# endernewton/tf-faster-rcnn

Hardware: AMD Instinct MI355X
Metric: images/sec (600×1000) ResNet-101 Faster R-CNN at 1/2/4/8 MI355X (higher is better)
Workload: dtype f32 (operands, accumulators, results; GEMMs with Cin, Cout % 128 == 0 form each f32 product from two-piece fp16 operands with an exact power-of-two scale per 128-k block on the fp16 matrix pipe -- 3 MFMAs / product, dropped terms <= 3 * 2^-22, measured error vs float64 below the f32-MFMA kernel's; o

## Files before the change

### include/frcnn_hip.h

```cpp
#ifndef FRCNN_HIP_H_
#define FRCNN_HIP_H_
#include <stddef.h>
#include <stdint.h>

#ifdef __cplusplus
extern "C" {
#endif

#define FRCNN_OK 0
#define FRCNN_E_ARG (-1)
#define FRCNN_E_WS (-2)
#define FRCNN_E_UNSUPPORTED (-3)
#define FRCNN_E_HIP(e) (-(1000 + (int)(e)))

#define FRCNN_NMS_RULE_CPU 0
#define FRCNN_NMS_RULE_GPU 1

#define FRCNN_ACT_NONE 0
#define FRCNN_ACT_RELU 1
#define FRCNN_ACT_RELU6 2

#define FRCNN_ABI_VERSION 6
int frcnn_abi_version(void);
const char* frcnn_build_info(void);
// ... 115 lines not shown
int frcnn_proposal_recall_host(const float* boxes, int box_stride, long long n_rows, const long long* start, const int* count,
                               const float* scale, int n_images, long long max_boxes, int limit, const double* gt,
                               const long long* gt_off, long long n_gt_total, double* gt_iou, int* ran_out, void* ws, size_t ws_bytes);

int frcnn_conv2d_nhwc(const float* x_d, int N, int H, int W, int Cin, const float* w_d, const float* bias_d,
                      const float* residual_d, int RH, int RW, int res_stride, float* y_d, int OH, int OW,
                      int Cout, int KH, int KW, int stride, int pad_top, int pad_left, int act, int fold_w,
                      void* stream);
size_t frcnn_conv2d_workspace_bytes(int N, int OH, int OW, int Cout, int KH, int KW, int Cin, int fold_w);
int frcnn_conv2d_nhwc_ws(const float* x_d, int N, int H, int W, int Cin, const float* w_d, const float* bias_d,
                         const float* residual_d, int RH, int RW, int res_stride, float* y_d, int OH, int OW, int Cout, int KH,
                         int KW, int stride, int pad_top, int pad_left, int act, int fold_w, void* ws, size_t ws_bytes,
                         void* stream);

int frcnn_set_tuning(int key, int value);
unsigned int frcnn_crc32c(const void* data, size_t n, unsigned int crc);

long long frcnn_snappy_uncompress(const unsigned char* src, size_t n, unsigned char* dst, size_t cap);

int frcnn_prep_image_shape(int h, int w, int target_size, int max_size, double* im_scale, int* out_h, int* out_w);
int frcnn_prep_image(const void* src_d, int src_is_float, int h, int w, const double* pixel_means, double im_scale, float* out_d,
                     int OH, int OW, int out_c, void* stream);
int frcnn_prep_image_batched(const void* src_d, int src_is_float, int B, int h, int w, const double* pixel_means, double im_scale,
                             float* out_d, int OH, int OW, int out_c, void* stream);
int frcnn_prep_train_image(const void* src_d, int src_is_float, int h, int w, int flipped, const double* pixel_means, double im_scale,
                           float* out_d, int OH, int OW, int out_c, const unsigned short* boxes_d, const int* classes_d, int G,
                           float* gt_d, void* stream);

int frcnn_jpeg_info(const unsigned char* data, size_t n, int* out8);
size_t frcnn_jpeg_coef_bytes(int width, int height, int ncomp, int hs, int vs);
int frcnn_jpeg_entropy_decode(const unsigned char* data, size_t n, void* coef_h, size_t coef_bytes);
int frcnn_jpeg_pixels_host(const void* coef_h, int width, int height, int ncomp, int hs, int vs, unsigned char* bgr_h);
size_t frcnn_jpeg_workspace_bytes(int width, int height, int ncomp, int hs, int vs);
int frcnn_jpeg_pixels(const void* coef_d, int width, int height, int ncomp, int hs, int vs, unsigned char* bgr_d, void* ws,
                      size_t ws_bytes, void* stream);

int frcnn_jpeg_quant_tables(int quality, unsigned short* out128);
int frcnn_jpeg_coefs(const unsigned char* bgr_d, int width, int height, int hs, int vs, int quality, void* coef_d, void* ws,
                     size_t ws_bytes, void* stream);
int frcnn_jpeg_coefs_host(const unsigned char* bgr_h, int width, int height, int hs, int vs, int quality, void* coef_h);
size_t frcnn_jpeg_stream_bound(int width, int height, int hs, int vs);
long long frcnn_jpeg_entropy_encode(const void* coef_h, int width, int height, int hs, int vs, unsigned char* out, size_t cap);

int frcnn_draw_detections(unsigned char* bgr_d, int h, int w, const float* dets_d, const int* cnt_d, int max_dets, float conf,
                          int thickness, int scale, const unsigned char* colours_d, int num_colours, const unsigned char* labels_d,
                          int num_classes, int label_stride, const unsigned char* glyphs_d, void* stream);
int frcnn_draw_detections_host(unsigned char* bgr_h, int h, int w, const float* dets_h, int count, int max_dets, float conf,
                               int thickness, int scale, const unsigned char* colours_h, int num_colours, const unsigned char* labels_h,
                               int num_classes, int label_stride, const unsigned char* glyphs_h);

int frcnn_gemm_batched_nt(const float* x_d, const float* w_d, float* y_d, int G, int M, int N, int K, void* stream);
size_t frcnn_gemm_x3_pack_bytes(int G, int N, int K);
int frcnn_gemm_x3_pack(const float* w_d, int G, int N, int K, void* planes_d, void* stream);
int frcnn_gemm_x3(const float* x_d, const void* planes_d, const float* bias_d, const float* res_d, float* y_d, int G, int M, int N,
                  int K, int act, int cfg, int terms, void* stream);
size_t frcnn_h2_planes_bytes(long long rows, int K);
int frcnn_h2_pack_w(const float* w_d, int G, int N, int K, void* planes_d, float* w_inv_d, void* stream);
int frcnn_h2_split(const float* x_d, long long M, int K, void* planes_d, float* inv_d, void* stream);
int frcnn_gemm_h2(const void* x_planes_d, const float* x_inv_d, const void* w_planes_d, const float* w_inv_d, const float* bias_d,
                  const float* res_d, const void* res_planes_d, const float* res_inv_d, float* y_d, void* y_planes_d, float* y_inv_d,
                  int G, int M, int N, int K, int act, int cfg, void* stream);
size_t frcnn_gemm_h2_mean_workspace_bytes(int G, int M, int N);
int frcnn_gemm_h2_mean(const void* x_planes_d, const float* x_inv_d, const void* w_planes_d, const float* w_inv_d, const float* bias_d,
                       const float* res_d, const void* res_planes_d, const float* res_inv_d, int G, int M, int N, int K, int act, int rows,
                       float* mean_out_d, void* ws, size_t ws_bytes, int cfg, void* stream);
int frcnn_winograd_filter_transform(const float* w_hwio, int Cin, int Cout, const float* scale, int m, float* u_out);
int frcnn_winograd_filter_transform_device(const float* w_packed_d, int Cout, int Cin, int m, int transpose_flip, float* u_d,
                                           void* stream);
int frcnn_winograd_input_transform(const float* x_d, int N, int H, int W, int C, int m, float* v_d, void* stream);
int frcnn_winograd_output_transform(const float* m_d, int N, int H, int W, int C, int m, const float* bias_d, int act, float* y_d,
                                    void* stream);
int frcnn_winograd2_conv_x3(const float* x_d, int N, int H, int W, const void* u_planes_d, const float* bias_d, int act, float* y_d,
                            void* stream);
int frcnn_winograd7_filter_transform(const float* w_hwio, int Cin, int Cout, const float* scale, float* u_out);
int frcnn_winograd7_filter_transform_device(const float* w_packed_d, int Cout, int Cin, int transpose_flip, float* u_d, void* stream);
int frcnn_winograd7_input_transform(const float* x_d, int R, int C, float* v_d, void* stream);
int frcnn_winograd7_output_transform(const float* m_d, int R, int C, const float* bias_d, int act, float* y_d, void* stream);
int frcnn_winograd_input_transform_h2(const float* x_d, int N, int H, int W, int C, int m, void* v_planes_d, float* v_inv_d, void* stream);
int frcnn_winograd_output_transform_h2(const float* m_d, int N, int H, int W, int C, int m, const float* bias_d, int act, float* y_d,
                                       void* y_planes_d, float* y_inv_d, void* stream);
int frcnn_winograd7_input_transform_h2(const float* x_d, int R, int C, void* v_planes_d, float* v_inv_d, void* stream);
int frcnn_winograd7_output_transform_h2(const float* m_d, int R, int C, const float* bias_d, int act, float* y_d, void* y_planes_d,
                                        float* y_inv_d, void* stream);
int frcnn_pack_filter_hwio(const float* w_hwio, int KH, int KW, int Cin, int Cout, const float* scale, float* out);
int frcnn_maxpool_nhwc(const float* x_d, int N, int H, int W, int C, int k, int stride, int pad_top,
                       int pad_left, float* y_d, int OH, int OW, void* stream);
int frcnn_dwconv3x3_nhwc(const float* x_d, int N, int H, int W, int C, const float* w_d, const float* bias_d,
                         float* y_d, int OH, int OW, int stride, int pad_top, int pad_left, int act, void* stream);
int frcnn_dwconv3x3_nhwc_h2(const float* x_d, int N, int H, int W, int C, const float* w_d, const float* bias_d, float* y_d,
                            void* y_planes_d, float* y_inv_d, int OH, int OW, int stride, int pad_top, int pad_left, int act, void* stream);
int frcnn_spatial_mean(const float* x_d, int N, int HW, int C, float* y_d, void* stream);
int frcnn_softmax_rows(const float* x_d, int R, int C, int ld, float* y_d, void* stream);
int frcnn_rpn_softmax(const float* score_d, int HW, int A, int ld, float* prob_d, void* stream);
int frcnn_copy_cols(const float* src_d, int R, int ld_src, int col0, int cols, float* dst_d, int ld_dst, void* stream);

size_t frcnn_anchor_target_workspace_bytes(int H, int W, int A, int max_gt);
int frcnn_anchor_target_layer(const float* gt_boxes_d, int G, float im_h, float im_w, int H, int W, int A,
                              int feat_stride, const double* base_d, int rpn_batchsize, double fg_fraction,
                              double pos_overlap, double neg_overlap, long long seed, const double* opts, float* labels_d,
                              float* bbox_targets_d, float* inside_w_d, float* outside_w_d, void* ws,
                              size_t ws_bytes, void* stream);
int frcnn_anchor_target_layer_inject(const float* gt_boxes_d, int G, float im_h, float im_w, int H, int W, int A, int feat_stride,
                                     const double* base_d, int rpn_batchsize, double fg_fraction, double pos_overlap,
                                     double neg_overlap, const int* disable_d, int n_disable, const double* opts, float* labels_d,
                                     float* bbox_targets_d, float* inside_w_d, float* outside_w_d, void* ws, size_t ws_bytes,
                                     void* stream);
int frcnn_proposal_target_layer(const float* rpn_rois_d, const float* rpn_scores_d, int N, const float* gt_boxes_d,
                                int G, int num_classes, int batch_size, double fg_fraction, double fg_thresh,
                                double bg_thresh_hi, double bg_thresh_lo, const double* means4, const double* stds4,
                                long long seed, const double* opts, float* rois_d, float* roi_scores_d, float* labels_d,
                                float* bbox_targets_d, float* inside_w_d, float* outside_w_d, int* counts_d,
                                void* stream);
int frcnn_proposal_target_layer_dn(const float* rpn_rois_d, const float* rpn_scores_d, int max_rois, const int* num_rois_d,
                                   const float* gt_boxes_d, int G, int num_classes, int batch_size, double fg_fraction,
                                   double fg_thresh, double bg_thresh_hi, double bg_thresh_lo, const double* means4,
                                   const double* stds4, long long seed, const double* opts, float* rois_d, float* roi_scores_d,
                                   float* labels_d, float* bbox_targets_d, float* inside_w_d, float* outside_w_d, int* counts_d,
                                   void* stream);
int frcnn_proposal_target_layer_inject(const float* rpn_rois_d, const float* rpn_scores_d, int N, const float* gt_boxes_d, int G,
                                       int num_classes, int batch_size, const int* keep_inds_d, int n_fg, const double* means4,
                                       const double* stds4, const double* opts, float* rois_d, float* roi_scores_d, float* labels_d,
                                       float* bbox_targets_d, float* inside_w_d, float* outside_w_d, void* stream);
size_t frcnn_loss_workspace_bytes(long long elements);
int frcnn_softmax_ce_loss(const float* logits_d, const float* labels_d, int R, int C, int rpn_A, int rpn_H, int rpn_W,
                          float* loss_d, float* dlogits_d, void* ws, size_t ws_bytes, void* stream);
int frcnn_smooth_l1_loss(const float* pred_d, const float* targets_d, const float* inside_w_d, const float* outside_w_d,
                         long long n, float sigma, float mean_divisor, float* loss_d, float* dpred_d, void* ws,
                         size_t ws_bytes, void* stream);

int frcnn_transpose_pad(const float* in_d, int M, int C, float* out_d, int Mp, void* stream);
int frcnn_im2col_t(const float* x_d, int N, int H, int W, int Cin, int OH, int OW, int KH, int KW, int stride,
                   int pad_top, int pad_left, float* out_d, int Mp, void* stream);
int frcnn_flip_transpose_filter(const float* w_d, int Cout, int KH, int KW, int Cin, float* out_d, void* stream);
int frcnn_conv2d_dgrad_strided(const float* dy_d, int N, int OH, int OW, int Cout, const float* w_d, int KH, int KW,
                               int Cin, int stride, int pad_top, int pad_left, float* dx_d, int H, int W,
                               int accumulate, void* stream);
int frcnn_conv2d_wgrad_supported(int Cin, int Cout);
size_t frcnn_conv2d_wgrad_workspace_bytes(int N, int OH, int OW, int Cin, int Cout, int KH, int KW);
int frcnn_conv2d_wgrad(const float* dy_d, const float* x_d, int N, int H, int W, int Cin, int OH, int OW, int Cout, int KH, int KW,
                       int stride, int pad_top, int pad_left, float* dw_d, void* ws, size_t ws_bytes, void* stream);
void frcnn_conv2d_wgrad_set_plan(int tile, int min_workgroups);
size_t frcnn_conv2d_wgrad_h2_workspace_bytes(int N, int OH, int OW, int Cin, int Cout, int KH, int KW);
int frcnn_conv2d_wgrad_h2(const float* dy_d, const float* x_d, int N, int H, int W, int Cin, int OH, int OW, int Cout, int KH, int KW,
                          int stride, int pad_top, int pad_left, float* dw_d, void* ws, size_t ws_bytes, void* stream);
void frcnn_conv2d_wgrad_h2_set_plan(int tile, int min_workgroups);
int frcnn_relu_bwd(float* grad_d, const float* y_d, long long n, void* stream);
int frcnn_conv2d_nhwc_masked_ws(const float* x_d, int N, int H, int W, int Cin, const float* w_d, const float* bias_d,
                                const float* residual_d, int RH, int RW, int res_stride, float* y_d, int OH, int OW,
                                int Cout, int KH, int KW, int stride, int pad_top, int pad_left, int act, const float* mask_d,
                                void* ws, size_t ws_bytes, void* stream);
int frcnn_gemm_h2_masked(const void* x_planes_d, const float* x_inv_d, const void* w_planes_d, const float* w_inv_d, const float* bias_d,
                         const float* res_d, const float* mask_d, float* y_d, void* y_planes_d, float* y_inv_d, int G, int M, int N, int K,
                         int act, int cfg, void* stream);
int frcnn_winograd_output_transform_masked(const float* m_d, int N, int H, int W, int C, int m, const float* mask_d, float* y_d,
                                           void* y_planes_d, float* y_inv_d, void* stream);
int frcnn_winograd7_output_transform_masked(const float* m_d, int R, int C, const float* mask_d, float* y_d, void* y_planes_d,
                                            float* y_inv_d, void* stream);
int frcnn_relu6_bwd(float* grad_d, const float* y_d, long long n, void* stream);
int frcnn_maxpool_bwd(const float* x_d, int N, int H, int W, int C, int k, int stride, const float* y_d, const float* dy_d,
                      int OH, int OW, float* dx_d, void* stream);
int frcnn_dropout(const float* x_d, long long n, unsigned long long seed, float keep_prob, float* y_d, void* stream);
int frcnn_dwconv3x3_dgrad(const float* g_d, int N, int OH, int OW, int C, const float* w_d, float* dx_d, int H, int W, int stride,
                          int pad_top, int pad_left, int accumulate, void* stream);
size_t frcnn_dwconv3x3_wgrad_workspace_bytes(int N, int OH, int OW, int C);
int frcnn_dwconv3x3_wgrad(const float* g_d, const float* x_d, int N, int H, int W, int C, int OH, int OW, int stride, int pad_top,
                          int pad_left, const float* scale_d, float* dw_d, void* ws, size_t ws_bytes, void* stream);
// ... 41 lines not shown
```

### tf-faster-rcnn_amd/csrc/conv_igemm.hip

```cpp
#include "common.h"
#include "mfma_f32.h"
#include <mutex>
#include <type_traits>

__device__ float4 g_zero_page[4];

struct ConvParams {
  const float* x; const float* w; const float* bias; const float* res; float* y;
  const float* mask;
  int N, H, W, Cin, OH, OW, Cout, KH, KW, stride, pad_top, pad_left, act;
  int RH, RW, res_stride;
  int M, Ktot, nsteps;
  int mtiles, ntiles;
  int batch;
  long long gx, gw, gy;
  int reserved;
  int splits, kchunk;
  long long gz;
  int stagger, stagger_slots;
};

__device__ __forceinline__ size_t res_offset_strided(int m, int n, int Cout, int res_stride, int ohow, int OW, int RH, int RW) {
  const int img = m / ohow, rem = m % ohow, oh = rem / OW, ow = rem % OW;
  return ((size_t)(img * RH + oh * res_stride) * RW + ow * res_stride) * Cout + n;
// ... 449 lines not shown
    if (last) {
      next = __builtin_amdgcn_readfirstlane(tile + W8);
      set_tile(next < t_end ? next : tile);
      prefetch_res();
    }
    slab_body(cur);
    cur ^= 1;
    if (!last) { ++step; continue; }
    if (p.res) finish(std::true_type{}); else finish(std::false_type{});
    if (next >= t_end) break;
    zero_acc();
    step = 0; tile = next; c_bm0 = i_bm0; c_bn0 = i_bn0; c_g = i_g;
  }
  wait_vmcnt<0>();
}

template <int BM, int BN, int WM, int WN, bool ILV, bool RF, bool RESPF>
static int launch_stream(const ConvParams& c, hipStream_t st) {
  constexpr int NT = (BM / WM) * (BN / WN) * 64;
  constexpr size_t lds = sizeof(float) * 2 * (BM + BN) * 32;
  auto kern = k_gemm_stream<BM, BN, WM, WN, ILV, RF, RESPF>;
  static KernelOnce once;
  int slots = 0;
  HIP_TRY(kernel_once(once, (const void*)kern, NT, lds, &slots));
  const bool plain = c.KH == 1 && c.KW == 1 && c.stride == 1 && c.pad_top == 0 && c.pad_left == 0 && c.OH == c.H && c.OW == c.W;
  if (slots < 8 || !plain || c.mask || c.Cout % BN || c.splits != 1 || (c.res && c.res_stride != 1) || (long long)c.M * c.Cout >= (1ll << 31) ||
      (long long)c.M * c.Cin >= (1ll << 31) || (long long)c.Cout * c.Cin >= (1ll << 31))
    return FRCNN_E_UNSUPPORTED;
  GemmParams p;
  p.x = c.x; p.w = c.w; p.bias = c.bias; p.res = c.res; p.y = c.y;
  p.mtiles = cdiv(c.M, BM); p.M = c.M; p.N = c.Cout; p.K = c.Cin; p.nsteps = c.Cin / 32;
  p.ntiles = c.Cout / BN; p.batch = c.batch; p.act = c.act;
  p.gx = c.gx; p.gw = c.gw; p.gy = c.gy;
  const long long T = (long long)p.mtiles * p.ntiles * p.batch;
  if (T >= (1ll << 30)) return FRCNN_E_UNSUPPORTED;
  const int grid = (int)min((long long)(slots / 8) * 8, ((T + 7) / 8) * 8);
  hipLaunchKernelGGL(kern, dim3(grid), dim3(NT), lds, st, p);
  LAUNCH_CHECK();
  return FRCNN_OK;
}

enum : int {
  IGEMM_64x32_NS4 = 4,
  IGEMM_64x64_ILV = 15,
  IGEMM_128_RF = 20,
  IGEMM_128_8W_RF = 21,
  STREAM_64x64 = 100, STREAM_64x64_RESPF = 101,
  STREAM_128_RF = 102,
  STREAM_128_8W_RF = 104, STREAM_128_8W_RF_RESPF = 105,
  STREAM_128x64 = 106, STREAM_128x64_RESPF = 107,
  STREAM_64x128 = 108, STREAM_64x128_RESPF = 109,
  STREAM_128x64_4W_RESPF = 110, STREAM_64x128_4W_RESPF = 111,
  STREAM_32x64 = 112,
  STREAM_32x128 = 114,
};

static int launch_cfg(int id, const ConvParams& p, hipStream_t st) {
  switch (id) {
    case IGEMM_64x32_NS4: return launch_conv<64, 32, 32, 32, 4, false>(p, st);
    case IGEMM_64x64_ILV: return launch_conv<64, 64, 32, 32, 2, false, true>(p, st);
    case IGEMM_128_RF: return launch_conv<128, 128, 64, 64, 2, false, false, true>(p, st);
    case IGEMM_128_8W_RF: return launch_conv<128, 128, 32, 64, 2, false, false, true>(p, st);
    case STREAM_64x64: return launch_stream<64, 64, 32, 32, true, false, false>(p, st);
    case STREAM_64x64_RESPF: return launch_stream<64, 64, 32, 32, true, false, true>(p, st);
    case STREAM_128_RF: return launch_stream<128, 128, 64, 64, false, true, false>(p, st);
    case STREAM_128_8W_RF: return launch_stream<128, 128, 32, 64, false, true, false>(p, st);
    case STREAM_128_8W_RF_RESPF: return launch_stream<128, 128, 32, 64, false, true, true>(p, st);
    case STREAM_128x64: return launch_stream<128, 64, 32, 32, true, false, false>(p, st);
    case STREAM_128x64_RESPF: return launch_stream<128, 64, 32, 32, true, false, true>(p, st);
    case STREAM_64x128: return launch_stream<64, 128, 32, 32, true, false, false>(p, st);
    case STREAM_64x128_RESPF: return launch_stream<64, 128, 32, 32, true, false, true>(p, st);
    case STREAM_128x64_4W_RESPF: return launch_stream<128, 64, 64, 32, false, true, true>(p, st);
    case STREAM_64x128_4W_RESPF: return launch_stream<64, 128, 32, 64, false, true, true>(p, st);
    case STREAM_32x64: return launch_stream<32, 64, 32, 32, true, false, false>(p, st);
    case STREAM_32x128: return launch_stream<32, 128, 32, 32, true, false, false>(p, st);
    default: return FRCNN_E_ARG;
  }
}

static thread_local int g_force_cfg = -1, g_stagger = 0, g_stream = 1, g_split_target = 640;
static thread_local int g_plan_images = 0;
static constexpr int PLAN_IMAGES = 4;
extern thread_local int g_wino_rows_below;
extern "C" int frcnn_set_tuning(int key, int value) {
  if (key == 9) { g_wino_rows_below = value > 0 ? value : 256; return FRCNN_OK; }
  if (key == 0) { g_force_cfg = value; return FRCNN_OK; }
  if (key == 5) { g_stagger = value; return FRCNN_OK; }
  if (key == 6) { g_stream = value; return FRCNN_OK; }
  if (key == 7) { g_split_target = value > 0 ? value : 640; return FRCNN_OK; }
  if (key == 8) { g_plan_images = value > 0 ? value : 0; return FRCNN_OK; }
  return FRCNN_E_ARG;
}

static long long plan_rows(long long M) {
  return (g_plan_images > 0 && M % g_plan_images == 0) ? M / g_plan_images * PLAN_IMAGES : M;
}

static long long tiles_128(long long rows, int Cout, int groups) { return (rows + 127) / 128 * cdiv(Cout, 128) * groups; }

static int tile_cfg_64(int Cout) { return Cout > 32 ? IGEMM_64x64_ILV : IGEMM_64x32_NS4; }
static int tile_cfg(long long rows, int Cout, int nsteps, int groups) {
  if (Cout >= 96 && tiles_128(rows, Cout, groups) >= 384 && nsteps >= 8) return Cout >= 1024 ? IGEMM_128_8W_RF : IGEMM_128_RF;
  return tile_cfg_64(Cout);
}

static bool short_k_stream(long long rows, int Cout, int nsteps, int groups) {
  return g_stream && nsteps <= 8 && Cout % 128 == 0 && (rows + 63) / 64 * (Cout / 128) * groups >= 512;
}

static int plan_splits(int M, int Cout, int nsteps) {
  if (g_force_cfg >= 0) return 1;
  M = (int)min(plan_rows(M), (long long)0x7fffffff);
  if (tile_cfg(M, Cout, nsteps, 1) != tile_cfg_64(Cout)) return 1;
  const long long tiles = (long long)cdiv(M, 64) * cdiv(Cout, Cout > 32 ? 64 : 32);
  if (tiles >= 384 || nsteps < 16) return 1;
  int S = (int)min((long long)8, (g_split_target + tiles - 1) / tiles);
  S = min(S, nsteps / 8);
  if (S < 2) return 1;
  const int kchunk = cdiv(nsteps, S);
  return cdiv(nsteps, kchunk);
}

extern "C" size_t frcnn_conv2d_workspace_bytes(int N, int OH, int OW, int Cout, int KH, int KW, int Cin, int fold_w) {
  if (fold_w || N <= 0 || OH <= 0 || OW <= 0 || Cout <= 0 || KH <= 0 || KW <= 0 || Cin <= 0 || Cin % 32) return 0;
  const long long M = (long long)N * OH * OW;
  if (M >= (1ll << 29)) return 0;
  const int S = plan_splits((int)M, Cout, KH * KW * (Cin / 32));
  return S > 1 ? (size_t)S * (size_t)M * (size_t)Cout * sizeof(float) : 0;
}

__global__ void k_splitk_finish(const float* __restrict__ part, int S, int M, int Cout, const float* __restrict__ bias,
                                const float* res, int res_stride, int OH, int OW, int RH, int RW, int act, const float* __restrict__ mask,
                                float* y) {
  const long long total = (long long)M * Cout;
  const int ohow = OH * OW;
  for (long long i = (long long)blockIdx.x * blockDim.x + threadIdx.x; i < total; i += (long long)gridDim.x * blockDim.x) {
    float v = part[i];
    for (int s = 1; s < S; ++s) v += part[(size_t)s * total + i];
    const int m = (int)(i / Cout), n = (int)(i - (long long)m * Cout);
    if (bias) v += bias[n];
    if (res) {
      size_t ro;
      if (res_stride == 1) ro = (size_t)i;
      else ro = res_offset_strided(m, n, Cout, res_stride, ohow, OW, RH, RW);
      v += res[ro];
    }
    if (act == FRCNN_ACT_RELU) v = act_relu(v);
    else if (act == FRCNN_ACT_RELU6) v = act_relu6(v);
    if (mask) v = mask[i] > 0.f ? v : 0.f;
    y[i] = v;
  }
}

static ConvParams conv_params() {
  ConvParams p = {};
  p.KH = p.KW = p.stride = p.res_stride = p.batch = p.splits = 1;
  p.act = FRCNN_ACT_NONE;
  return p;
}

static int conv2d_impl(const float* x_d, int N, int H, int W, int Cin, const float* w_d, const float* bias_d,
                       const float* residual_d, int RH, int RW, int res_stride, float* y_d, int OH, int OW, int Cout, int KH, int KW,
                       int stride, int pad_top, int pad_left, int act, int fold_w, void* ws, size_t ws_bytes, const float* mask_d,
                       void* stream) {
  if (!x_d || !w_d || !y_d) return FRCNN_E_ARG;
  if (N <= 0 || H <= 0 || W <= 0 || Cin <= 0 || OH <= 0 || OW <= 0 || Cout <= 0 || KH <= 0 || KW <= 0 || stride <= 0)
    return FRCNN_E_ARG;
// ... 111 lines not shown
```

### tf-faster-rcnn_amd/csrc/detect_kernels.hip

```cpp
#include "common.h"
#include "softnms_math.h"
#include "boxvote_math.h"

extern "C" int frcnn_generate_anchors(int base_size, const double* ratios, int n_ratios, const double* scales,
                                      int n_scales, double* out_base) {
  if (!ratios || !scales || !out_base || n_ratios <= 0 || n_scales <= 0 || base_size <= 0) return FRCNN_E_ARG;
  const double w = (double)base_size, h = (double)base_size;
  const double cx = 0.5 * (w - 1), cy = 0.5 * (h - 1);
  for (int r = 0; r < n_ratios; ++r) {
    const double ws = nearbyint(sqrt(w * h / ratios[r]));
    const double hs = nearbyint(ws * ratios[r]);
    const double x1 = cx - 0.5 * (ws - 1), y1 = cy - 0.5 * (hs - 1);
    const double x2 = cx + 0.5 * (ws - 1), y2 = cy + 0.5 * (hs - 1);
    const double aw = x2 - x1 + 1, ah = y2 - y1 + 1;
    const double acx = x1 + 0.5 * (aw - 1), acy = y1 + 0.5 * (ah - 1);
    for (int s = 0; s < n_scales; ++s) {
      const double sw = aw * scales[s], sh = ah * scales[s];
      double* o = out_base + 4 * ((size_t)r * n_scales + s);
      o[0] = acx - 0.5 * (sw - 1);
      o[1] = acy - 0.5 * (sh - 1);
      o[2] = acx + 0.5 * (sw - 1);
      o[3] = acy + 0.5 * (sh - 1);
    }
  }
  return FRCNN_OK;
}

__device__ __forceinline__ float4 anchor_at(const double* __restrict__ base, int n, int A, int W, int stride) {
  const int a = n % A, pix = n / A;
  const double sx = (double)((pix % W) * stride), sy = (double)((pix / W) * stride);
  const double* b = base + 4 * a;
  return make_float4((float)(b[0] + sx), (float)(b[1] + sy), (float)(b[2] + sx), (float)(b[3] + sy));
}

__global__ void k_anchors(const double* __restrict__ base, int A, int W, int stride, int N, float4* __restrict__ out) {
  const int n = blockIdx.x * blockDim.x + threadIdx.x;
  if (n < N) out[n] = anchor_at(base, n, A, W, stride);
}

extern "C" int frcnn_generate_anchors_pre(int height, int width, int feat_stride, const double* base_d, int A,
                                          float* anchors_d, void* stream) {
  if (!base_d || !anchors_d || height <= 0 || width <= 0 || A <= 0) return FRCNN_E_ARG;
  const int N = height * width * A;
  hipLaunchKernelGGL(k_anchors, dim3(cdiv(N, 256)), dim3(256), 0, (hipStream_t)stream, base_d, A, width,
                     feat_stride, N, (float4*)anchors_d);
  LAUNCH_CHECK();
  return FRCNN_OK;
}

#define NMS_RULE_CPU FRCNN_NMS_RULE_CPU
#define NMS_RULE_GPU FRCNN_NMS_RULE_GPU
#define NMS_RULE_TF 2

__global__ void k_decode_clip_key(const float* __restrict__ prob, const float4* __restrict__ deltas,
                                  const double* __restrict__ base, int A, int W, int stride, int N, float hi_x,
                                  float hi_y, float4* __restrict__ boxes, u64* __restrict__ keys, size_t img) {
  const int n = blockIdx.x * blockDim.x + threadIdx.x;
  if (n >= N) return;
  const int b = blockIdx.y;
  prob += (size_t)b * 2 * N;
  deltas += (size_t)b * N;
  const int a = n % A, pix = n / A;
  const float score = prob[(size_t)pix * 2 * A + A + a];
  float4 bx = decode_box(anchor_at(base, n, A, W, stride), deltas[n]);
  bx.x = rmax(rmin(bx.x, hi_x), 0.0f);
  bx.y = rmax(rmin(bx.y, hi_y), 0.0f);
  bx.z = rmax(rmin(bx.z, hi_x), 0.0f);
  bx.w = rmax(rmin(bx.w, hi_y), 0.0f);
  img_ptr(boxes, img, b)[n] = bx;
  img_ptr(keys, img, b)[n] = make_key(score, (u32)n);
}

__global__ void k_dets_key(const float* __restrict__ dets, int k, float4* __restrict__ boxes, u64* __restrict__ keys) {
  const int n = blockIdx.x * blockDim.x + threadIdx.x;
  if (n >= k) return;
  const float* d = dets + 5 * (size_t)n;
  boxes[n] = make_float4(d[0], d[1], d[2], d[3]);
  keys[n] = make_key(d[4], (u32)n);
}

__global__ void k_boxes_scores_key(const float4* __restrict__ in_boxes, const float* __restrict__ in_scores, int k,
                                   float4* __restrict__ boxes, u64* __restrict__ keys) {
  const int n = blockIdx.x * blockDim.x + threadIdx.x;
  if (n >= k) return;
  boxes[n] = in_boxes[n];
// ... 652 lines not shown
  if (!rpn_cls_prob_d || !rpn_bbox_pred_d || !base_d || !rois_d || !scores_d || !ws) return FRCNN_E_ARG;
  if (H <= 0 || W <= 0 || A <= 0 || rpn_top_n <= 0) return FRCNN_E_ARG;
  const int N = H * W * A;
  if (N < rpn_top_n) return FRCNN_E_UNSUPPORTED;
  hipStream_t st = (hipStream_t)stream;
  SortWs s = carve(ws, N, rpn_top_n);
  if (s.bytes > ws_bytes) return FRCNN_E_WS;
  int rc = launch_decode(s, rpn_cls_prob_d, rpn_bbox_pred_d, 1, im_h, im_w, W, A, feat_stride, base_d, N, st);
  if (rc) return rc;
  rc = launch_topk_sort(s, N, rpn_top_n, 1, st);
  if (rc) return rc;
  hipLaunchKernelGGL(k_top_rois, dim3(cdiv(rpn_top_n, 256)), dim3(256), 0, st, s.sboxes, s.sscores, rpn_top_n, rois_d,
                     scores_d);
  LAUNCH_CHECK();
  return FRCNN_OK;
}

extern "C" int frcnn_proposal_top_layer_inds(const float* rpn_cls_prob_d, const float* rpn_bbox_pred_d, float im_h, float im_w,
                                             int H, int W, int A, int feat_stride, const double* base_d, const int* top_inds_d,
                                             int n_inds, float* rois_d, float* scores_d, void* stream) {
  if (!rpn_cls_prob_d || !rpn_bbox_pred_d || !base_d || !rois_d || !scores_d || !top_inds_d) return FRCNN_E_ARG;
  if (H <= 0 || W <= 0 || A <= 0 || n_inds <= 0) return FRCNN_E_ARG;
  hipLaunchKernelGGL(k_decode_gather, dim3(cdiv(n_inds, 256)), dim3(256), 0, (hipStream_t)stream, rpn_cls_prob_d,
                     (const float4*)rpn_bbox_pred_d, base_d, A, W, feat_stride, H * W * A, im_w - 1.0f, im_h - 1.0f, top_inds_d, n_inds,
                     rois_d, scores_d);
  LAUNCH_CHECK();
  return FRCNN_OK;
}

extern "C" int frcnn_non_max_suppression(const float* boxes_d, const float* scores_d, int k, int max_output_size,
                                         float iou_threshold, int* selected_d, int* num_d, void* ws, size_t ws_bytes,
                                         void* stream) {
  if (!num_d || k < 0 || max_output_size < 0) return FRCNN_E_ARG;
  hipStream_t st = (hipStream_t)stream;
  if (k == 0 || max_output_size == 0) {
    HIP_TRY(hipMemsetAsync(num_d, 0, sizeof(int), st));
    return FRCNN_OK;
  }
  if (!boxes_d || !scores_d || !selected_d || !ws) return FRCNN_E_ARG;
  if (k > NMS_MAX_BOXES) return FRCNN_E_UNSUPPORTED;
  SortWs s = carve(ws, k, k);
  if (s.bytes > ws_bytes) return FRCNN_E_WS;
  hipLaunchKernelGGL(k_boxes_scores_key, dim3(cdiv(k, 256)), dim3(256), 0, st, (const float4*)boxes_d, scores_d, k, s.boxes,
                     s.keys);
  LAUNCH_CHECK();
  int rc = launch_topk_sort(s, k, k, 1, st);
  if (rc) return rc;
  rc = launch_mask(s, k, 1, iou_threshold, NMS_RULE_TF, st);
  if (rc) return rc;
  ReduceOut o = {s.sboxes, s.sscores, s.sidx, nullptr, nullptr, selected_d, num_d, 0};
  return launch_reduce(s, k, 1, min(max_output_size, k), o, st);
}

extern "C" int frcnn_proposal_layer_tf_batched(const float* rpn_cls_prob_d, const float* rpn_bbox_pred_d, int B, float im_h,
                                               float im_w, int H, int W, int A, int feat_stride, const double* base_d,
                                               int post_nms_topn, float nms_thresh, float* rois_d, float* scores_d, int* num_d,
                                               void* ws, size_t ws_bytes, void* stream) {
  if (!rpn_cls_prob_d || !rpn_bbox_pred_d || !base_d || !rois_d || !scores_d || !num_d || !ws) return FRCNN_E_ARG;
  if (B <= 0 || H <= 0 || W <= 0 || A <= 0 || post_nms_topn <= 0) return FRCNN_E_ARG;
  const long long NN = (long long)H * W * A;
  if (NN > NMS_MAX_BOXES) return FRCNN_E_UNSUPPORTED;
  const int N = (int)NN;
  hipStream_t st = (hipStream_t)stream;
  SortWs s = carve(ws, N, N);
  if (s.bytes * (size_t)B > ws_bytes) return FRCNN_E_WS;
  int rc = launch_decode(s, rpn_cls_prob_d, rpn_bbox_pred_d, B, im_h, im_w, W, A, feat_stride, base_d, N, st);
  if (rc) return rc;
  rc = launch_topk_sort(s, N, N, B, st);
  if (rc) return rc;
  rc = launch_mask(s, N, B, nms_thresh, NMS_RULE_TF, st);
  if (rc) return rc;
  ReduceOut o = {s.sboxes, s.sscores, s.sidx, rois_d, scores_d, nullptr, num_d, 1};
  return launch_reduce(s, N, B, post_nms_topn, o, st);
}

extern "C" int frcnn_proposal_layer_tf(const float* rpn_cls_prob_d, const float* rpn_bbox_pred_d, float im_h, float im_w,
                                       int H, int W, int A, int feat_stride, const double* base_d, int post_nms_topn,
                                       float nms_thresh, float* rois_d, float* scores_d, int* num_d, void* ws,
                                       size_t ws_bytes, void* stream) {
  return frcnn_proposal_layer_tf_batched(rpn_cls_prob_d, rpn_bbox_pred_d, 1, im_h, im_w, H, W, A, feat_stride, base_d, post_nms_topn,
                                         nms_thresh, rois_d, scores_d, num_d, ws, ws_bytes, stream);
}

__device__ __forceinline__ float4 lerp4(const float4 a, const float4 b, float t) {
  return make_float4(a.x + (b.x - a.x) * t, a.y + (b.y - a.y) * t, a.z + (b.z - a.z) * t, a.w + (b.w - a.w) * t);
}
__device__ __forceinline__ float4 max4(const float4 a, const float4 b) {
  return make_float4(fmaxf(a.x, b.x), fmaxf(a.y, b.y), fmaxf(a.z, b.z), fmaxf(a.w, b.w));
}

__device__ __forceinline__ float4 crop_sample(const float4* __restrict__ feat, int H, int W, int C4, int c4, float y1,
                                              float x1, float hs, float ws, int gy, int gx) {
  const float in_y = y1 * (float)(H - 1) + (float)gy * hs;
  const float in_x = x1 * (float)(W - 1) + (float)gx * ws;
  if (in_y < 0 || in_y > (float)(H - 1) || in_x < 0 || in_x > (float)(W - 1)) return make_float4(0, 0, 0, 0);
  const int top = (int)floorf(in_y), bot = (int)ceilf(in_y);
  const int left = (int)floorf(in_x), right = (int)ceilf(in_x);
  const float ly = in_y - (float)top, lx = in_x - (float)left;
  const float4 tl = feat[((size_t)top * W + left) * C4 + c4], tr = feat[((size_t)top * W + right) * C4 + c4];
  const float4 bl = feat[((size_t)bot * W + left) * C4 + c4], br = feat[((size_t)bot * W + right) * C4 + c4];
  return lerp4(lerp4(tl, tr, lx), lerp4(bl, br, lx), ly);
}

template <bool MAX2>
__global__ __launch_bounds__(256) void k_crop_and_resize(const float4* __restrict__ feat_all, int NIMG, int H, int W, int C4,
                                                         int nslab, const float* __restrict__ rois, float stride, int pool,
                                                         const float4* __restrict__ bias, int act, float4* __restrict__ out) {
  const int slab = blockIdx.x % nslab, rp = blockIdx.x / nslab;
  const int r = rp / pool, py = rp % pool;
  const int SC4 = C4 / nslab, c40 = slab * SC4;
  const float height = ((float)H - 1.0f) * stride, width = ((float)W - 1.0f) * stride;
  const float* roi = rois + 5 * (size_t)r;
  const int img = (int)roi[0];
  float4* orow = out + ((size_t)r * pool + py) * pool * C4;
  if (img < 0 || img >= NIMG) {
    for (int t = threadIdx.x; t < pool * SC4; t += 256) orow[(size_t)(t / SC4) * C4 + c40 + t % SC4] = make_float4(0, 0, 0, 0);
    return;
  }
  const float4* feat = feat_all + (size_t)img * H * W * C4;
  const float x1 = roi[1] / width, y1 = roi[2] / height, x2 = roi[3] / width, y2 = roi[4] / height;
  const int P = MAX2 ? 2 * pool : pool;
  const float hs = (y2 - y1) * (float)(H - 1) / (float)(P - 1);
  const float ws = (x2 - x1) * (float)(W - 1) / (float)(P - 1);
  for (int t = threadIdx.x; t < pool * SC4; t += 256) {
    const int px = t / SC4, c4 = c40 + t % SC4;
    float4 v;
    if (MAX2) {
      v = crop_sample(feat, H, W, C4, c4, y1, x1, hs, ws, 2 * py, 2 * px);
      v = max4(v, crop_sample(feat, H, W, C4, c4, y1, x1, hs, ws, 2 * py, 2 * px + 1));
      v = max4(v, crop_sample(feat, H, W, C4, c4, y1, x1, hs, ws, 2 * py + 1, 2 * px));
      v = max4(v, crop_sample(feat, H, W, C4, c4, y1, x1, hs, ws, 2 * py + 1, 2 * px + 1));
    } else {
      v = crop_sample(feat, H, W, C4, c4, y1, x1, hs, ws, py, px);
    }
    if (bias) {
      const float4 bv = bias[c4];
      v.x += bv.x; v.y += bv.y; v.z += bv.z; v.w += bv.w;
    }
    if (act == FRCNN_ACT_RELU) v = act_relu(v);
    orow[(size_t)px * C4 + c4] = v;
  }
}

template <bool MAX2, int ITEMS>
__global__ __launch_bounds__(256) void k_crop_and_resize_roi(const float4* __restrict__ feat_all, int NIMG, int H, int W, int C4,
                                                             int nslab, const float* __restrict__ rois, float stride, int pool,
                                                             const float4* __restrict__ bias, int act, float4* __restrict__ out) {
  const int slab = blockIdx.x % nslab, r = blockIdx.x / nslab;
  const int SC4 = C4 / nslab, c40 = slab * SC4;
  const float height = ((float)H - 1.0f) * stride, width = ((float)W - 1.0f) * stride;
  const float* roi = rois + 5 * (size_t)r;
  const int img = (int)roi[0];
  float4* obase = out + (size_t)r * pool * pool * C4;
  const int total = pool * pool * SC4;
  if (img < 0 || img >= NIMG) {
    for (int t = threadIdx.x; t < total; t += 256) obase[(size_t)(t / SC4) * C4 + c40 + t % SC4] = make_float4(0, 0, 0, 0);
    return;
  }
  const float4* feat = feat_all + (size_t)img * H * W * C4;
  const float x1 = roi[1] / width, y1 = roi[2] / height, x2 = roi[3] / width, y2 = roi[4] / height;
  const int P = MAX2 ? 2 * pool : pool;
  const float hs = (y2 - y1) * (float)(H - 1) / (float)(P - 1);
  const float ws = (x2 - x1) * (float)(W - 1) / (float)(P - 1);
  for (int t0 = threadIdx.x; t0 < total; t0 += 256 * ITEMS) {
    float4 v[ITEMS];
#pragma unroll
    for (int k = 0; k < ITEMS; ++k) {
      const int t = t0 + k * 256;
      if (t >= total) { v[k] = make_float4(0, 0, 0, 0); continue; }
      const int pix = t / SC4, c4 = c40 + t % SC4;
      const int py = pix / pool, px = pix - py * pool;
      if (MAX2) {
        v[k] = crop_sample(feat, H, W, C4, c4, y1, x1, hs, ws, 2 * py, 2 * px);
        v[k] = max4(v[k], crop_sample(feat, H, W, C4, c4, y1, x1, hs, ws, 2 * py, 2 * px + 1));
        v[k] = max4(v[k], crop_sample(feat, H, W, C4, c4, y1, x1, hs, ws, 2 * py + 1, 2 * px));
        v[k] = max4(v[k], crop_sample(feat, H, W, C4, c4, y1, x1, hs, ws, 2 * py + 1, 2 * px + 1));
      } else {
        v[k] = crop_sample(feat, H, W, C4, c4, y1, x1, hs, ws, py, px);
      }
    }
#pragma unroll
    for (int k = 0; k < ITEMS; ++k) {
      const int t = t0 + k * 256;
      if (t >= total) continue;
      const int pix = t / SC4, c4 = c40 + t % SC4;
      float4 o = v[k];
      if (bias) {
        const float4 bv = bias[c4];
        o.x += bv.x; o.y += bv.y; o.z += bv.z; o.w += bv.w;
      }
      if (act == FRCNN_ACT_RELU) o = act_relu(o);
      obase[(size_t)pix * C4 + c4] = o;
    }
  }
}

static thread_local int g_crop_slabs = -1;
static thread_local int g_crop_form = 0;

static int launch_crop(const float* feat_d, int NIMG, int H, int W, int C, const float* rois_d, int R, float feat_stride, int pool,
                       int fuse_max2x2, const float* bias_d, int act, float* out_d, void* stream) {
  if (R == 0) return FRCNN_OK;
  if (!feat_d || !rois_d || !out_d || NIMG <= 0 || H < 2 || W < 2 || C <= 0 || R < 0 || pool < 2) return FRCNN_E_ARG;
  if (C % 4) return FRCNN_E_UNSUPPORTED;
  hipStream_t st = (hipStream_t)stream;
  const int C4 = C / 4;
  int nslab = (C4 % 8 == 0 && C4 / 8 >= 16) ? 8 : 1;
  if (g_crop_form == 0 && nslab == 8 && C4 / 8 < 32) nslab = 4;
  if (g_crop_slabs > 0 && C4 % g_crop_slabs == 0) nslab = g_crop_slabs;
  const long long blocks = (long long)R * pool * nslab;
  if (blocks >= (1ll << 31)) return FRCNN_E_UNSUPPORTED;
  if (g_crop_form == 0) {
    const unsigned grid = (unsigned)((long long)R * nslab);
    if (fuse_max2x2)
      hipLaunchKernelGGL((k_crop_and_resize_roi<true, 2>), dim3(grid), dim3(256), 0, st, (const float4*)feat_d, NIMG, H, W, C4, nslab, rois_d,
                         feat_stride, pool, (const float4*)bias_d, act, (float4*)out_d);
    else
      hipLaunchKernelGGL((k_crop_and_resize_roi<false, 4>), dim3(grid), dim3(256), 0, st, (const float4*)feat_d, NIMG, H, W, C4, nslab, rois_d,
                         feat_stride, pool, (const float4*)bias_d, act, (float4*)out_d);
    LAUNCH_CHECK();
    return FRCNN_OK;
  }
  if (fuse_max2x2)
    hipLaunchKernelGGL(k_crop_and_resize<true>, dim3((unsigned)blocks), dim3(256), 0, st, (const float4*)feat_d, NIMG, H, W, C4, nslab,
                       rois_d, feat_stride, pool, (const float4*)bias_d, act, (float4*)out_d);
  else
    hipLaunchKernelGGL(k_crop_and_resize<false>, dim3((unsigned)blocks), dim3(256), 0, st, (const float4*)feat_d, NIMG, H, W, C4, nslab,
                       rois_d, feat_stride, pool, (const float4*)bias_d, act, (float4*)out_d);
  LAUNCH_CHECK();
  return FRCNN_OK;
}

extern "C" int frcnn_detect_set_tuning(int key, int value) {
  if (key == 4) { g_crop_slabs = value; return FRCNN_OK; }
  if (key == 5) { g_crop_form = value; return FRCNN_OK; }
  return FRCNN_E_ARG;
}

extern "C" int frcnn_crop_and_resize(const float* feat_d, int H, int W, int C, const float* rois_d, int R,
                                     float feat_stride, int pool, int fuse_max2x2, float* out_d, void* stream) {
  return launch_crop(feat_d, 1, H, W, C, rois_d, R, feat_stride, pool, fuse_max2x2, nullptr, FRCNN_ACT_NONE, out_d, stream);
}

extern "C" int frcnn_crop_and_resize_batched(const float* feat_d, int N, int H, int W, int C, const float* rois_d, int R,
                                             float feat_stride, int pool, int fuse_max2x2, float* out_d, void* stream) {
  return launch_crop(feat_d, N, H, W, C, rois_d, R, feat_stride, pool, fuse_max2x2, nullptr, FRCNN_ACT_NONE, out_d, stream);
// ... 755 lines not shown
```

### tf-faster-rcnn_amd/csrc/gemm_h2.hip

```cpp
#include "h2_common.h"
#include <mutex>
#include <type_traits>

typedef float f32x16 __attribute__((ext_vector_type(16)));
typedef _Float16 h8 __attribute__((ext_vector_type(8)));

#define LDS_AS __attribute__((address_space(3)))

struct GemmH2Params {
  const unsigned short* x; const float* x_inv; const unsigned short* w; const float* w_inv;
  const float* bias; const float* res; const unsigned short* resp; const float* resp_inv; float* y; unsigned short* yp; float* y_inv;
  int M, N, K, batch, act, nsteps, mtiles, ntiles;
  long long Mtot;
  int wshare;
  const float* mask;
  float* mean_part; int mean_rows;
};

__device__ __forceinline__ void h2_glds16(unsigned voff, const void* sbase, unsigned lds_base) {
  unsigned keep;
  asm volatile(
      "s_mov_b32 %0, m0\n\t"
      "s_mov_b32 m0, %3\n\t"
      "s_nop 0\n\t"
// ... 1050 lines not shown
  const long long T = (long long)p.mtiles * p.ntiles * p.batch;
  if (T >= (1ll << 30)) return FRCNN_E_UNSUPPORTED;
  const int grid = (int)min((long long)(slots / 8) * 8, ((T + 7) / 8) * 8);
  hipLaunchKernelGGL(kern, dim3(grid), dim3(NT), lds, st, p);
  LAUNCH_CHECK();
  return FRCNN_OK;
}

template <int MASK>
static int h2_dispatch(const GemmH2Params& p, int cfg, hipStream_t st) {
  switch (cfg) {
    case 9: return launch_h2<128, 128, 64, 64, 2, 2, H2_SCALES_ONCE + MASK>(p, st);
    case 12: return launch_h2<64, 128, 32, 64, 2, 2, MASK>(p, st);
    case 21: return launch_h2<256, 128, 64, 64, 3, 2, H2_SCALES_ONCE + H2_PINGPONG + MASK>(p, st);
    case 30: return launch_h2<128, 128, 64, 64, 2, 2, H2_SCALES_ONCE + H2_LIGHT_BOUNDARY + MASK>(p, st);
    case 31: return launch_h2<128, 128, 64, 64, 2, 2, H2_SCALES_ONCE + H2_LIGHT_BOUNDARY + H2_STORE16 + MASK>(p, st);
    case 32: return launch_h2<128, 128, 64, 64, 2, 2, H2_SCALES_ONCE + H2_STORE16 + MASK>(p, st);
    case 33: return launch_h2<64, 128, 32, 64, 2, 2, H2_LIGHT_BOUNDARY + H2_STORE16 + MASK>(p, st);
    case 34: return launch_h2<256, 128, 64, 64, 3, 2, H2_SCALES_ONCE + H2_PINGPONG + H2_STORE16 + MASK>(p, st);
    case 40: return launch_h2<128, 128, 64, 64, 2, 2, H2_SCALES_ONCE + H2_LIGHT_BOUNDARY + H2_STORE16 + H2_DEFERRED + MASK>(p, st);
    case 41: return launch_h2<64, 128, 32, 64, 2, 2, H2_LIGHT_BOUNDARY + H2_STORE16 + H2_DEFERRED + MASK>(p, st);
  }
#ifdef FRCNN_ABLATION
  constexpr int CFG31 = H2_SCALES_ONCE + H2_LIGHT_BOUNDARY + H2_STORE16;
  if constexpr (MASK == 0) switch (cfg) {
    case 50: return launch_h2<128, 128, 64, 64, 2, 2, CFG31 + H2_NO_MFMA>(p, st);
    case 51: return launch_h2<128, 128, 64, 64, 2, 2, CFG31 + H2_NO_FRAG>(p, st);
    case 52: return launch_h2<128, 128, 64, 64, 2, 2, CFG31 + H2_NO_LOAD>(p, st);
    case 53: return launch_h2<128, 128, 64, 64, 2, 2, CFG31 + H2_NO_MFMA + H2_NO_FRAG>(p, st);
    case 54: return launch_h2<128, 128, 64, 64, 2, 2, CFG31 + H2_NO_FRAG + H2_NO_LOAD>(p, st);
    case 55: return launch_h2<128, 128, 64, 64, 2, 2, CFG31 + H2_NO_MFMA + H2_NO_FRAG + H2_NO_LOAD>(p, st);
  }
#endif
  return FRCNN_E_ARG;
}

static int run_h2(GemmH2Params& p, int cfg, hipStream_t st);
#ifndef FRCNN_H2_PP_CLASSES
#define FRCNN_H2_PP_CLASSES 7
#endif

static GemmH2Params h2_params(const void* x_planes_d, const float* x_inv_d, const void* w_planes_d, const float* w_inv_d, const float* bias_d,
                              const float* res_d, const void* res_planes_d, const float* res_inv_d, float* y_d, void* y_planes_d, float* y_inv_d,
                              int G, int M, int N, int K, int act) {
  GemmH2Params p;
  p.x = (const unsigned short*)x_planes_d; p.x_inv = x_inv_d; p.w = (const unsigned short*)w_planes_d; p.w_inv = w_inv_d;
  p.bias = bias_d; p.res = res_d; p.resp = (const unsigned short*)res_planes_d; p.resp_inv = res_inv_d; p.y = y_d; p.yp = (unsigned short*)y_planes_d; p.y_inv = y_inv_d;
  p.M = M; p.N = N; p.K = K; p.batch = G; p.act = act; p.Mtot = (long long)G * M;
  p.nsteps = p.mtiles = p.ntiles = 0;
  p.mean_part = nullptr; p.mean_rows = 0; p.wshare = 0; p.mask = nullptr;
  return p;
}

extern "C" int frcnn_gemm_h2(const void* x_planes_d, const float* x_inv_d, const void* w_planes_d, const float* w_inv_d, const float* bias_d,
                             const float* res_d, const void* res_planes_d, const float* res_inv_d, float* y_d, void* y_planes_d, float* y_inv_d,
                             int G, int M, int N, int K, int act, int cfg, void* stream) {
  if (!x_planes_d || !x_inv_d || !w_planes_d || !w_inv_d || (!y_d && !y_planes_d) || (y_planes_d && !y_inv_d) || G <= 0 || M <= 0 || N <= 0 ||
      K <= 0 || act < 0 || act > 2 || (res_d && res_planes_d) || (res_planes_d && !res_inv_d))
    return FRCNN_E_ARG;
  const long long Mtot = (long long)G * M;
  if (K % H2_KB || N % 128 || 4ll * Mtot * K >= (1ll << 32) || 4ll * N * K >= (1ll << 32) ||
      (long long)M * N >= (1ll << 29))
    return FRCNN_E_UNSUPPORTED;
  GemmH2Params p = h2_params(x_planes_d, x_inv_d, w_planes_d, w_inv_d, bias_d, res_d, res_planes_d, res_inv_d, y_d, y_planes_d, y_inv_d, G, M, N, K, act);
  return run_h2(p, cfg, (hipStream_t)stream);
}

extern "C" int frcnn_gemm_h2_masked(const void* x_planes_d, const float* x_inv_d, const void* w_planes_d, const float* w_inv_d, const float* bias_d,
                                    const float* res_d, const float* mask_d, float* y_d, void* y_planes_d, float* y_inv_d, int G, int M, int N, int K,
                                    int act, int cfg, void* stream) {
  if (!x_planes_d || !x_inv_d || !w_planes_d || !w_inv_d || !mask_d || (!y_d && !y_planes_d) || (y_planes_d && !y_inv_d) || G <= 0 || M <= 0 ||
      N <= 0 || K <= 0 || act < 0 || act > 2)
    return FRCNN_E_ARG;
  const long long Mtot = (long long)G * M;
  if (K % H2_KB || N % 128 || 4ll * Mtot * K >= (1ll << 32) || 4ll * N * K >= (1ll << 32) || (long long)M * N >= (1ll << 29)) return FRCNN_E_UNSUPPORTED;
  GemmH2Params p = h2_params(x_planes_d, x_inv_d, w_planes_d, w_inv_d, bias_d, res_d, nullptr, nullptr, y_d, y_planes_d, y_inv_d, G, M, N, K, act);
  p.mask = mask_d;
  return run_h2(p, cfg, (hipStream_t)stream);
}

static int run_h2(GemmH2Params& p, int cfg, hipStream_t st) {
  const int G = p.batch, M = p.M, N = p.N, K = p.K;
  if (cfg < 0) {
    const bool classes = cfg == -1;
    if (cfg == -9) cfg = -1;
    const long long mt256 = (M + 255) / 256, t256 = mt256 * (N / 128) * G;
#ifndef FRCNN_H2_PP_MIN_K
#define FRCNN_H2_PP_MIN_K 1024
#endif
    const int pp_min_k = ((cfg == -4 || cfg == -5 || cfg == -6) && !p.mean_part) ? 512 : FRCNN_H2_PP_MIN_K;
    int pp_cfg = (cfg == -3 || cfg == -4 || (cfg == -6 && K < FRCNN_H2_PP_MIN_K)) ? 34 : 21;
    const bool waste256_ok = mt256 * 256 * 100 <= (long long)M * 104;
    bool pp = K >= pp_min_k && waste256_ok && t256 >= 256;
    bool to31 = false;
    if (classes && !p.mean_part && !p.mask) {
      const long long m64 = (M + 63) / 64 * 64;
      const bool waste64_ok = m64 * 100 <= (long long)M * 104;
      const bool products = (FRCNN_H2_PP_CLASSES & 1) && G > 1 && p.y && !p.yp && !p.res && !p.resp && K >= 512 && waste64_ok && t256 >= 256;
      const bool conv3_f32res = (FRCNN_H2_PP_CLASSES & 2) && p.res && p.yp && K == 512 && waste64_ok && t256 >= 256;
      if (conv3_f32res && !pp) pp_cfg = 34;
      pp = pp || products || conv3_f32res;
      to31 = (FRCNN_H2_PP_CLASSES & 4) && p.resp && p.yp && !p.y && K == 512;
    }
    const bool tiny = (long long)((M + 127) / 128) * (N / 128) * G < 150;
    const bool de = cfg != -2 && cfg != -7 && !p.mean_part && !p.mask && ((p.resp && p.yp && !p.y) || cfg == -8) && !to31;
    cfg = pp ? pp_cfg : tiny ? (cfg == -2 ? 12 : (de && cfg == -8) ? 41 : 33) : (cfg == -2 ? 9 : de ? 40 : 31);
  }
  if (p.mean_part && (cfg == 40 || cfg == 41)) cfg = cfg == 40 ? 31 : 33;
  return p.mask ? h2_dispatch<H2_MASKED>(p, cfg, st) : h2_dispatch<0>(p, cfg, st);
}

__global__ __launch_bounds__(256) void k_h2_mean_finish(const float* __restrict__ part, int G, int M, int N4, int rows, float4* __restrict__ out) {
  const long long t = (long long)blockIdx.x * blockDim.x + threadIdx.x;
  const int per = M / rows;
  if (t >= (long long)G * per * N4) return;
  const int n4 = (int)(t % N4);
  const long long gr = t / N4;
  const int g = (int)(gr / per), r = (int)(gr % per);
  const int nblk = (M + 31) >> 5;
  const int row0 = r * rows, row1 = row0 + rows - 1;
  float4 s = make_float4(0.f, 0.f, 0.f, 0.f);
  for (int b = row0 >> 5; b <= (row1 >> 5); ++b) {
    const int which = ((b << 5) / rows == r) ? 0 : 1;
    const float4 v = *(const float4*)(part + (((size_t)g * nblk + b) * 2 + which) * (size_t)N4 * 4 + (size_t)n4 * 4);
    s.x += v.x; s.y += v.y; s.z += v.z; s.w += v.w;
  }
  const float inv = 1.0f / (float)rows;
  out[t] = make_float4(s.x * inv, s.y * inv, s.z * inv, s.w * inv);
}

extern "C" size_t frcnn_gemm_h2_mean_workspace_bytes(int G, int M, int N) {
  if (G <= 0 || M <= 0 || N <= 0) return 256;
  return (size_t)G * (size_t)((M + 31) / 32) * 2 * (size_t)N * sizeof(float);
}

extern "C" int frcnn_gemm_h2_mean(const void* x_planes_d, const float* x_inv_d, const void* w_planes_d, const float* w_inv_d, const float* bias_d,
                                  const float* res_d, const void* res_planes_d, const float* res_inv_d, int G, int M, int N, int K, int act, int rows,
                                  float* mean_out_d, void* ws, size_t ws_bytes, int cfg, void* stream) {
  if (!x_planes_d || !x_inv_d || !w_planes_d || !w_inv_d || !mean_out_d || !ws || G <= 0 || M <= 0 || N <= 0 || K <= 0 || act < 0 || act > 2 ||
      rows <= 0 || (res_d && res_planes_d) || (res_planes_d && !res_inv_d))
    return FRCNN_E_ARG;
  const long long Mtot = (long long)G * M;
  if (K % H2_KB || N % 128 || M % rows || rows < 32 || 4ll * Mtot * K >= (1ll << 32) || 4ll * N * K >= (1ll << 32) || (long long)M * N >= (1ll << 29))
    return FRCNN_E_UNSUPPORTED;
  if (frcnn_gemm_h2_mean_workspace_bytes(G, M, N) > ws_bytes) return FRCNN_E_WS;
  GemmH2Params p = h2_params(x_planes_d, x_inv_d, w_planes_d, w_inv_d, bias_d, res_d, res_planes_d, res_inv_d, nullptr, nullptr, nullptr, G, M, N, K, act);
  p.mean_part = (float*)ws; p.mean_rows = rows; p.wshare = 1;
  hipStream_t st = (hipStream_t)stream;
  const int rc = run_h2(p, cfg, st);
  if (rc) return rc;
  const long long tot = (long long)G * (M / rows) * (N / 4);
  hipLaunchKernelGGL(k_h2_mean_finish, dim3((unsigned)((tot + 255) / 256)), dim3(256), 0, st, (const float*)ws, G, M, N / 4, rows, (float4*)mean_out_d);
  LAUNCH_CHECK();
  return FRCNN_OK;
}
```

### tf-faster-rcnn_amd/csrc/winograd7.hip

```cpp
#include "h2_common.h"

namespace w7 {
constexpr float BT[11][9] = {
    {4.f, 0.f, -5.f, 0.f, 1.f, 0.f, 0.f, 0.f, 0.f},  {0.f, -4.f, -4.f, 1.f, 1.f, 0.f, 0.f, 0.f, 0.f}, {0.f, 4.f, -4.f, -1.f, 1.f, 0.f, 0.f, 0.f, 0.f},
    {0.f, -2.f, -1.f, 2.f, 1.f, 0.f, 0.f, 0.f, 0.f}, {0.f, 2.f, -1.f, -2.f, 1.f, 0.f, 0.f, 0.f, 0.f}, {0.f, 4.f, 0.f, -5.f, 0.f, 1.f, 0.f, 0.f, 0.f},
    {0.f, 0.f, 0.f, 0.f, 2.f, -1.f, -2.f, 1.f, 0.f}, {0.f, 0.f, 0.f, 0.f, 0.f, -2.f, -1.f, 1.f, 0.f}, {0.f, 0.f, 0.f, 0.f, 0.f, 2.f, -3.f, 1.f, 0.f},
    {0.f, 0.f, 0.f, 0.f, 0.f, -1.f, 0.f, 1.f, 0.f},  {0.f, 0.f, 0.f, 0.f, 0.f, 2.f, -1.f, -2.f, 1.f}};
constexpr float AT[7][11] = {
    {1.f, 1.f, 1.f, 1.f, 1.f, 0.f, 0.f, 0.f, 0.f, 0.f, 0.f},  {0.f, 1.f, -1.f, 2.f, -2.f, 0.f, 0.f, 0.f, 0.f, 0.f, 0.f},
    {0.f, 1.f, 1.f, 4.f, 4.f, 0.f, 0.f, 0.f, 0.f, 0.f, 0.f},  {0.f, 1.f, -1.f, 8.f, -8.f, 1.f, 0.f, 0.f, 0.f, 0.f, 0.f},
    {0.f, 0.f, 0.f, 0.f, 0.f, 0.f, 1.f, 1.f, 1.f, 1.f, 0.f},  {0.f, 0.f, 0.f, 0.f, 0.f, 0.f, 0.f, 1.f, -1.f, 2.f, 0.f},
    {0.f, 0.f, 0.f, 0.f, 0.f, 0.f, 0.f, 1.f, 1.f, 4.f, 1.f}};
constexpr double G[11][3] = {{1.0 / 4, 0, 0},          {-1.0 / 6, -1.0 / 6, -1.0 / 6}, {-1.0 / 6, 1.0 / 6, -1.0 / 6}, {1.0 / 24, 1.0 / 12, 1.0 / 6},
                             {1.0 / 24, -1.0 / 12, 1.0 / 6}, {0, 0, 1},                {1.0 / 2, 0, 0},               {-1.0 / 2, -1.0 / 2, -1.0 / 2},
                             {-1.0 / 6, 1.0 / 6, -1.0 / 6},  {1.0 / 6, 1.0 / 3, 2.0 / 3}, {0, 0, 1}};
}

__device__ __forceinline__ float2 f2mad(float a, float2 x, float2 y) { return make_float2(a * x.x + y.x, a * x.y + y.y); }

__device__ __forceinline__ void acc_term(float2& acc, bool& first, float coef, const float2 x) {
  if (coef == 0.f) return;
  if (first) {
    acc = coef == 1.f ? x : (coef == -1.f ? make_float2(-x.x, -x.y) : make_float2(coef * x.x, coef * x.y));
    first = false;
  } else if (coef == 1.f) {
    acc = make_float2(acc.x + x.x, acc.y + x.y);
  } else if (coef == -1.f) {
    acc = make_float2(acc.x - x.x, acc.y - x.y);
  } else {
    acc = f2mad(coef, x, acc);
  }
}

template <bool H2>
struct Wino7Sink {
  float2* f; unsigned short* planes; float* inv; size_t rows;
  template <int NR>
  __device__ __forceinline__ void putn(const size_t* row, const float2* v, int c2, int C2) const {
    if (!H2 || f) {
#pragma unroll
      for (int n = 0; n < NR; ++n) f[row[n] * C2 + c2] = v[n];
    }
    if (H2) {
      size_t e[NR];
      float* slot[NR];
#pragma unroll
      for (int n = 0; n < NR; ++n) {
        e[n] = (row[n] * C2 + c2) * 2;
        slot[n] = inv + (size_t)(c2 >> 6) * rows + row[n];
      }
      h2_emit_rows64<NR>(v, e, slot, (1u << NR) - 1u, planes, rows * (size_t)C2 * 2, c2 & 63);
    }
  }
};

template <bool H2>
__global__ void __launch_bounds__(256) k_wino7_input(const float2* __restrict__ x, int R, int C2, const Wino7Sink<H2> V) {
  const long long id = (long long)blockIdx.x * blockDim.x + threadIdx.x;
  if (id >= (long long)R * C2) return;
  const int c2 = (int)(id % C2);
  const int r = (int)(id / C2);
  float2 d[7][7];
  const float2* src = x + (size_t)r * 49 * C2 + c2;
#pragma unroll
  for (int i = 0; i < 7; ++i)
#pragma unroll
    for (int j = 0; j < 7; ++j) d[i][j] = src[(size_t)(i * 7 + j) * C2];
#pragma unroll
  for (int xi = 0; xi < 11; ++xi) {
    float2 t[7];
#pragma unroll
    for (int j = 0; j < 7; ++j) {
      bool first = true;
      t[j] = make_float2(0.f, 0.f);
#pragma unroll
      for (int i = 0; i < 7; ++i) acc_term(t[j], first, w7::BT[xi][i + 1], d[i][j]);
    }
    float2 o[11];
    size_t rw[11];
#pragma unroll
    for (int nu = 0; nu < 11; ++nu) {
      bool first = true;
      float2 v = make_float2(0.f, 0.f);
#pragma unroll
      for (int j = 0; j < 7; ++j) acc_term(v, first, w7::BT[nu][j + 1], t[j]);
      o[nu] = v;
      rw[nu] = (size_t)(xi * 11 + nu) * R + r;
    }
    V.template putn<11>(rw, o, c2, C2);
  }
}

template <int XI0, int NXI, int I0, int NI, bool H2, bool MASK>
__device__ __forceinline__ void wino7_out_segment(const float2* __restrict__ in, size_t plane, float2 bv, int act, const Wino7Sink<H2>& y,
                                                  size_t row0, int c2, int C2, const float2* __restrict__ mask) {
  float2 m[NXI][11];
#pragma unroll
  for (int a = 0; a < NXI; ++a)
#pragma unroll
    for (int nu = 0; nu < 11; ++nu) m[a][nu] = in[(size_t)((XI0 + a) * 11 + nu) * plane];
#pragma unroll
  for (int i = 0; i < NI; ++i) {
    float2 s[11];
#pragma unroll
    for (int nu = 0; nu < 11; ++nu) {
      bool first = true;
      s[nu] = make_float2(0.f, 0.f);
#pragma unroll
      for (int a = 0; a < NXI; ++a) acc_term(s[nu], first, w7::AT[I0 + i][XI0 + a], m[a][nu]);
    }
    float2 o[7];
    size_t rw[7];
#pragma unroll
    for (int j = 0; j < 7; ++j) {
      bool first = true;
      float2 v = make_float2(0.f, 0.f);
#pragma unroll
      for (int nu = 0; nu < 11; ++nu) acc_term(v, first, w7::AT[j][nu], s[nu]);
      v = make_float2(v.x + bv.x, v.y + bv.y);
      if (act == FRCNN_ACT_RELU) v = act_relu(v);
      rw[j] = row0 + (I0 + i) * 7 + j;
      if (MASK) {
        const float2 k = mask[rw[j] * C2 + c2];
        v.x = k.x > 0.f ? v.x : 0.f; v.y = k.y > 0.f ? v.y : 0.f;
      }
      o[j] = v;
    }
    y.template putn<7>(rw, o, c2, C2);
  }
}

template <bool H2, bool MASK = false>
__global__ void __launch_bounds__(256) k_wino7_output(const float2* __restrict__ Mx, int R, int C2, const float2* __restrict__ bias, int act,
                                                       const float2* __restrict__ mask, const Wino7Sink<H2> y) {
  const long long id = (long long)blockIdx.x * blockDim.x + threadIdx.x;
  if (id >= (long long)R * C2) return;
  const int c2 = (int)(id % C2);
  const int r = (int)(id / C2);
  const size_t plane = (size_t)R * C2;
  const float2* in = Mx + (size_t)r * C2 + c2;
  const float2 bv = bias ? bias[c2] : make_float2(0.f, 0.f);
  wino7_out_segment<0, 6, 0, 4, H2, MASK>(in, plane, bv, act, y, (size_t)r * 49, c2, C2, mask);
  wino7_out_segment<6, 5, 4, 3, H2, MASK>(in, plane, bv, act, y, (size_t)r * 49, c2, C2, mask);
}

__global__ void k_wino7_filter(const float* __restrict__ w, int O, int C, int transpose_flip, float* __restrict__ U) {
  const long long id = (long long)blockIdx.x * blockDim.x + threadIdx.x;
  if (id >= (long long)O * C) return;
  int o, c;
  if (transpose_flip) { o = (int)(id % O); c = (int)(id / O); }
  else { c = (int)(id % C); o = (int)(id / C); }
  float g[3][3];
#pragma unroll
  for (int i = 0; i < 3; ++i)
#pragma unroll
    for (int j = 0; j < 3; ++j) {
      const int kh = transpose_flip ? 2 - i : i, kw = transpose_flip ? 2 - j : j;
      g[i][j] = w[(((size_t)o * 3 + kh) * 3 + kw) * C + c];
    }
  float t[11][3];
#pragma unroll
  for (int a = 0; a < 11; ++a)
#pragma unroll
    for (int j = 0; j < 3; ++j) t[a][j] = (float)w7::G[a][0] * g[0][j] + (float)w7::G[a][1] * g[1][j] + (float)w7::G[a][2] * g[2][j];
  const size_t plane = (size_t)O * C;
  float* out = U + (transpose_flip ? (size_t)c * O + o : (size_t)o * C + c);
#pragma unroll
  for (int a = 0; a < 11; ++a)
#pragma unroll
    for (int b = 0; b < 11; ++b)
      out[(size_t)(a * 11 + b) * plane] = t[a][0] * (float)w7::G[b][0] + t[a][1] * (float)w7::G[b][1] + t[a][2] * (float)w7::G[b][2];
}

extern "C" int frcnn_winograd7_filter_transform(const float* w_hwio, int Cin, int Cout, const float* scale, float* u_out) {
  if (!w_hwio || !u_out || Cin <= 0 || Cout <= 0) return FRCNN_E_ARG;
  for (int c = 0; c < Cin; ++c)
    for (int o = 0; o < Cout; ++o) {
      double g[3][3], t[11][3];
      const double sc = scale ? (double)scale[o] : 1.0;
      for (int i = 0; i < 3; ++i)
        for (int j = 0; j < 3; ++j) g[i][j] = (double)w_hwio[((size_t)(i * 3 + j) * Cin + c) * Cout + o] * sc;
      for (int a = 0; a < 11; ++a)
        for (int j = 0; j < 3; ++j) t[a][j] = w7::G[a][0] * g[0][j] + w7::G[a][1] * g[1][j] + w7::G[a][2] * g[2][j];
      for (int a = 0; a < 11; ++a)
        for (int b = 0; b < 11; ++b)
          u_out[((size_t)(a * 11 + b) * Cout + o) * Cin + c] = (float)(t[a][0] * w7::G[b][0] + t[a][1] * w7::G[b][1] + t[a][2] * w7::G[b][2]);
    }
  return FRCNN_OK;
}

extern "C" int frcnn_winograd7_filter_transform_device(const float* w_packed_d, int Cout, int Cin, int transpose_flip, float* u_d,
                                                       void* stream) {
  if (!w_packed_d || !u_d || Cout <= 0 || Cin <= 0) return FRCNN_E_ARG;
  const long long tot = (long long)Cout * Cin;
  hipLaunchKernelGGL(k_wino7_filter, dim3((unsigned)((tot + 255) / 256)), dim3(256), 0, (hipStream_t)stream, w_packed_d, Cout, Cin,
                     transpose_flip ? 1 : 0, u_d);
  LAUNCH_CHECK();
  return FRCNN_OK;
}

extern "C" int frcnn_winograd7_input_transform(const float* x_d, int R, int C, float* v_d, void* stream) {
  if (!x_d || !v_d || R <= 0 || C <= 0) return FRCNN_E_ARG;
  if (C % 2) return FRCNN_E_UNSUPPORTED;
  const long long tot = (long long)R * (C / 2);
  const Wino7Sink<false> sink{(float2*)v_d, nullptr, nullptr, 0};
  hipLaunchKernelGGL(k_wino7_input<false>, dim3((unsigned)((tot + 255) / 256)), dim3(256), 0, (hipStream_t)stream, (const float2*)x_d, R, C / 2, sink);
  LAUNCH_CHECK();
  return FRCNN_OK;
}

extern "C" int frcnn_winograd7_input_transform_h2(const float* x_d, int R, int C, void* v_planes_d, float* v_inv_d, void* stream) {
  if (!x_d || !v_planes_d || !v_inv_d || R <= 0 || C <= 0) return FRCNN_E_ARG;
  if (C % H2_KB) return FRCNN_E_UNSUPPORTED;
  const long long tot = (long long)R * (C / 2);
  const Wino7Sink<true> sink{nullptr, (unsigned short*)v_planes_d, v_inv_d, (size_t)121 * R};
  hipLaunchKernelGGL(k_wino7_input<true>, dim3((unsigned)((tot + 255) / 256)), dim3(256), 0, (hipStream_t)stream, (const float2*)x_d, R, C / 2, sink);
  LAUNCH_CHECK();
  return FRCNN_OK;
}

extern "C" int frcnn_winograd7_output_transform(const float* m_d, int R, int C, const float* bias_d, int act, float* y_d, void* stream) {
  if (!m_d || !y_d || R <= 0 || C <= 0) return FRCNN_E_ARG;
  if (C % 2 || (act != FRCNN_ACT_NONE && act != FRCNN_ACT_RELU)) return FRCNN_E_UNSUPPORTED;
  const long long tot = (long long)R * (C / 2);
  const Wino7Sink<false> sink{(float2*)y_d, nullptr, nullptr, 0};
  hipLaunchKernelGGL((k_wino7_output<false, false>), dim3((unsigned)((tot + 255) / 256)), dim3(256), 0, (hipStream_t)stream, (const float2*)m_d, R,
                     C / 2, (const float2*)bias_d, act, (const float2*)nullptr, sink);
  LAUNCH_CHECK();
  return FRCNN_OK;
}

extern "C" int frcnn_winograd7_output_transform_h2(const float* m_d, int R, int C, const float* bias_d, int act, float* y_d, void* y_planes_d,
                                                   float* y_inv_d, void* stream) {
  if (!m_d || !y_planes_d || !y_inv_d || R <= 0 || C <= 0) return FRCNN_E_ARG;
  if (C % H2_KB || (act != FRCNN_ACT_NONE && act != FRCNN_ACT_RELU)) return FRCNN_E_UNSUPPORTED;
  const long long tot = (long long)R * (C / 2);
  const Wino7Sink<true> sink{(float2*)y_d, (unsigned short*)y_planes_d, y_inv_d, (size_t)R * 49};
  hipLaunchKernelGGL((k_wino7_output<true, false>), dim3((unsigned)((tot + 255) / 256)), dim3(256), 0, (hipStream_t)stream, (const float2*)m_d, R,
                     C / 2, (const float2*)bias_d, act, (const float2*)nullptr, sink);
  LAUNCH_CHECK();
  return FRCNN_OK;
}

extern "C" int frcnn_winograd7_output_transform_masked(const float* m_d, int R, int C, const float* mask_d, float* y_d, void* y_planes_d,
                                                       float* y_inv_d, void* stream) {
  if (!m_d || !mask_d || (!y_d && !y_planes_d) || (y_planes_d && !y_inv_d) || R <= 0 || C <= 0) return FRCNN_E_ARG;
  if (C % 2 || (y_planes_d && C % H2_KB)) return FRCNN_E_UNSUPPORTED;
  const long long tot = (long long)R * (C / 2);
  if (y_planes_d) {
    const Wino7Sink<true> sink{(float2*)y_d, (unsigned short*)y_planes_d, y_inv_d, (size_t)R * 49};
    hipLaunchKernelGGL((k_wino7_output<true, true>), dim3((unsigned)((tot + 255) / 256)), dim3(256), 0, (hipStream_t)stream, (const float2*)m_d, R,
                       C / 2, (const float2*)nullptr, FRCNN_ACT_NONE, (const float2*)mask_d, sink);
  } else {
    const Wino7Sink<false> sink{(float2*)y_d, nullptr, nullptr, 0};
    hipLaunchKernelGGL((k_wino7_output<false, true>), dim3((unsigned)((tot + 255) / 256)), dim3(256), 0, (hipStream_t)stream, (const float2*)m_d, R,
                       C / 2, (const float2*)nullptr, FRCNN_ACT_NONE, (const float2*)mask_d, sink);
  }
  LAUNCH_CHECK();
  return FRCNN_OK;
}
```

### tf-faster-rcnn_amd/frcnn_hip/__init__.py

```python
import ctypes
import os
from ctypes import c_double, c_float, c_int, c_longlong, c_size_t, c_ulonglong, c_void_p

_PKG = os.path.dirname(os.path.abspath(__file__))
LIB_PATH = os.path.join(_PKG, "libfrcnn_hip.so")
_lib = None

ABI_VERSION = 6
ACT_NONE, ACT_RELU, ACT_RELU6 = 0, 1, 2
NMS_RULE_CPU, NMS_RULE_GPU = 0, 1

_P = c_void_p
SIGNATURES = {
    "frcnn_abi_version": (c_int, []),
    "frcnn_build_info": (ctypes.c_char_p, []),
    "_nms": (None, [_P, _P, _P, c_int, c_int, c_float, c_int]),
    "frcnn_nms_workspace_bytes": (c_size_t, [c_int]),
    "frcnn_nms": (c_int, [_P, c_int, c_double, c_int, _P, _P, _P, c_size_t, _P]),
    "frcnn_nms_sorted": (c_int, [_P, c_int, c_int, c_double, c_int, _P, _P, _P, c_size_t, _P]),
    "frcnn_nms_rule": (c_int, [_P, c_int, c_double, c_int, c_int, _P, _P, _P, c_size_t, _P]),
    "frcnn_nms_sorted_rule": (c_int, [_P, c_int, c_int, c_double, c_int, c_int, _P, _P, _P, c_size_t, _P]),
    "frcnn_generate_anchors": (c_int, [c_int, _P, c_int, _P, c_int, _P]),
    "frcnn_generate_anchors_pre": (c_int, [c_int, c_int, c_int, _P, c_int, _P, _P]),
    "frcnn_proposal_workspace_bytes": (c_size_t, [c_int, c_int, c_int, c_int]),
# ... 5 lines not shown
    "frcnn_proposal_top_layer_inds": (c_int, [_P, _P, c_float, c_float, c_int, c_int, c_int, c_int, _P, _P, c_int, _P, _P, _P]),
    "frcnn_proposal_layer_tf_batched": (c_int, [_P, _P, c_int, c_float, c_float, c_int, c_int, c_int, c_int, _P, c_int, c_float, _P, _P,
                                                _P, _P, c_size_t, _P]),
    "frcnn_proposal_top_layer": (c_int, [_P, _P, c_float, c_float, c_int, c_int, c_int, c_int, _P, c_int, _P, _P, _P,
                                         c_size_t, _P]),
    "frcnn_non_max_suppression": (c_int, [_P, _P, c_int, c_int, c_float, _P, _P, _P, c_size_t, _P]),
    "frcnn_proposal_layer_tf": (c_int, [_P, _P, c_float, c_float, c_int, c_int, c_int, c_int, _P, c_int, c_float, _P, _P, _P,
                                        _P, c_size_t, _P]),
    "frcnn_crop_and_resize": (c_int, [_P, c_int, c_int, c_int, _P, c_int, c_float, c_int, c_int, _P, _P]),
    "frcnn_crop_and_resize_batched": (c_int, [_P, c_int, c_int, c_int, c_int, _P, c_int, c_float, c_int, c_int, _P, _P]),
    "frcnn_crop_and_resize_bias_act": (c_int, [_P, c_int, c_int, c_int, c_int, _P, c_int, c_float, c_int, _P, c_int, _P, _P]),
    "frcnn_detect_set_tuning": (c_int, [c_int, c_int]),
    "frcnn_detect_post_batched_workspace_bytes": (c_size_t, [c_int, c_int, c_int]),
    "frcnn_detect_post_batched": (c_int, [_P, _P, _P, _P, c_int, c_int, c_int, c_double, c_int, c_int, c_double, c_int, c_float, c_int,
                                          _P, _P, c_int, c_longlong, _P, c_size_t, _P]),
    "frcnn_detect_post_soft_batched_workspace_bytes": (c_size_t, [c_int, c_int, c_int]),
    "frcnn_detect_post_soft_batched": (c_int, [_P, _P, _P, _P, c_int, c_int, c_int, c_double, c_int, c_int, c_double, c_int, c_float, c_int,
                                               c_int, c_double, c_float, _P, _P, c_int, c_longlong, _P, c_size_t, _P]),
    "frcnn_soft_nms": (c_int, [_P, c_int, c_double, c_int, c_int, c_double, c_float, _P, _P, _P, _P]),
    "frcnn_soft_nms_host": (c_int, [_P, c_int, c_double, c_int, c_int, c_double, c_float, _P, _P, _P]),
    "frcnn_detect_post_vote_batched_workspace_bytes": (c_size_t, [c_int, c_int, c_int]),
    "frcnn_detect_post_vote_batched": (c_int, [_P, _P, _P, _P, c_int, c_int, c_int, c_double, c_int, c_int, c_double, c_int, c_float, c_int,
                                               c_int, c_double, c_float, c_double, _P, _P, c_int, c_longlong, _P, c_size_t, _P]),
    "frcnn_box_vote": (c_int, [_P, c_int, _P, c_int, c_double, _P, _P]),
    "frcnn_box_vote_host": (c_int, [_P, c_int, _P, c_int, c_double, _P]),
    "frcnn_mirror_views": (c_int, [_P, c_int, c_int, c_int, c_int, _P, _P]),
    "frcnn_merge_flip_views": (c_int, [_P, _P, _P, _P, c_int, c_int, c_int, c_float, _P, _P, _P, _P, _P]),
    "frcnn_merge_flip_views_host": (c_int, [_P, _P, _P, _P, c_int, c_int, c_int, c_float, _P, _P, _P, _P]),
    "frcnn_detect_post_workspace_bytes": (c_size_t, [c_int, c_int]),
    "frcnn_detect_post": (c_int, [_P, _P, _P, _P, c_int, c_int, c_double, c_int, c_int, c_double, c_float, c_int, _P, _P,
                                  c_int, _P, c_size_t, _P]),
    "frcnn_im_detect_boxes": (c_int, [_P, _P, c_int, c_int, c_double, c_int, c_int, _P, _P]),
    "frcnn_bbox_overlaps": (c_int, [_P, c_int, _P, c_int, _P, _P]),
    "frcnn_coco_match_workspace_bytes": (c_size_t, [c_int, c_longlong, c_longlong, c_longlong]),
    "frcnn_coco_match": (c_int, [_P, _P, _P, _P, _P, _P, c_int, _P, c_int, _P, c_int, _P, _P, _P, _P, _P, c_size_t, _P]),
    "frcnn_proposal_recall_workspace_bytes": (c_size_t, [c_int, c_longlong, c_longlong]),
    "frcnn_proposal_recall": (c_int, [_P, c_int, c_longlong, _P, _P, _P, c_int, c_longlong, c_int, _P, _P, c_longlong, _P, _P, _P, c_size_t, _P]),
    "frcnn_proposal_recall_host": (c_int, [_P, c_int, c_longlong, _P, _P, _P, c_int, c_longlong, c_int, _P, _P, c_longlong, _P, _P, _P, c_size_t]),
    "frcnn_bbox_transform_inv": (c_int, [_P, _P, c_int, c_int, _P, _P]),
    "frcnn_clip_boxes": (c_int, [_P, c_int, c_int, c_float, c_float, _P]),
    "frcnn_bbox_transform": (c_int, [_P, _P, c_int, _P, _P]),
    "frcnn_conv2d_nhwc": (c_int, [_P, c_int, c_int, c_int, c_int, _P, _P, _P, c_int, c_int, c_int, _P, c_int, c_int,
                                  c_int, c_int, c_int, c_int, c_int, c_int, c_int, c_int, _P]),
    "frcnn_conv2d_workspace_bytes": (c_size_t, [c_int, c_int, c_int, c_int, c_int, c_int, c_int, c_int]),
    "frcnn_conv2d_nhwc_ws": (c_int, [_P, c_int, c_int, c_int, c_int, _P, _P, _P, c_int, c_int, c_int, _P, c_int, c_int,
                                     c_int, c_int, c_int, c_int, c_int, c_int, c_int, c_int, _P, c_size_t, _P]),
    "frcnn_conv2d_nhwc_masked_ws": (c_int, [_P, c_int, c_int, c_int, c_int, _P, _P, _P, c_int, c_int, c_int, _P, c_int, c_int,
                                            c_int, c_int, c_int, c_int, c_int, c_int, c_int, _P, _P, c_size_t, _P]),
    "frcnn_gemm_h2_masked": (c_int, [_P, _P, _P, _P, _P, _P, _P, _P, _P, _P, c_int, c_int, c_int, c_int, c_int, c_int, _P]),
    "frcnn_winograd_output_transform_masked": (c_int, [_P, c_int, c_int, c_int, c_int, c_int, _P, _P, _P, _P, _P]),
    "frcnn_winograd7_output_transform_masked": (c_int, [_P, c_int, c_int, _P, _P, _P, _P, _P]),
    "frcnn_crc32c": (ctypes.c_uint32, [_P, c_size_t, ctypes.c_uint32]),
    "frcnn_snappy_uncompress": (c_longlong, [_P, c_size_t, _P, c_size_t]),
    "frcnn_prep_image_shape": (c_int, [c_int, c_int, c_int, c_int, _P, _P, _P]),
    "frcnn_prep_image": (c_int, [_P, c_int, c_int, c_int, _P, c_double, _P, c_int, c_int, c_int, _P]),
    "frcnn_prep_image_batched": (c_int, [_P, c_int, c_int, c_int, c_int, _P, c_double, _P, c_int, c_int, c_int, _P]),
    "frcnn_prep_train_image": (c_int, [_P, c_int, c_int, c_int, c_int, _P, c_double, _P, c_int, c_int, c_int, _P, _P, c_int, _P, _P]),
    "frcnn_jpeg_info": (c_int, [_P, c_size_t, _P]),
    "frcnn_jpeg_coef_bytes": (c_size_t, [c_int, c_int, c_int, c_int, c_int]),
    "frcnn_jpeg_entropy_decode": (c_int, [_P, c_size_t, _P, c_size_t]),
    "frcnn_jpeg_pixels_host": (c_int, [_P, c_int, c_int, c_int, c_int, c_int, _P]),
    "frcnn_jpeg_workspace_bytes": (c_size_t, [c_int, c_int, c_int, c_int, c_int]),
    "frcnn_jpeg_pixels": (c_int, [_P, c_int, c_int, c_int, c_int, c_int, _P, _P, c_size_t, _P]),
    "frcnn_jpeg_quant_tables": (c_int, [c_int, _P]),
    "frcnn_jpeg_coefs": (c_int, [_P, c_int, c_int, c_int, c_int, c_int, _P, _P, c_size_t, _P]),
    "frcnn_jpeg_coefs_host": (c_int, [_P, c_int, c_int, c_int, c_int, c_int, _P]),
    "frcnn_jpeg_stream_bound": (c_size_t, [c_int, c_int, c_int, c_int]),
    "frcnn_jpeg_entropy_encode": (c_longlong, [_P, c_int, c_int, c_int, c_int, _P, c_size_t]),
    "frcnn_draw_detections": (c_int, [_P, c_int, c_int, _P, _P, c_int, c_float, c_int, c_int, _P, c_int, _P, c_int, c_int, _P, _P]),
    "frcnn_draw_detections_host": (c_int, [_P, c_int, c_int, _P, c_int, c_int, c_float, c_int, c_int, _P, c_int, _P, c_int, c_int, _P]),
    "frcnn_gemm_batched_nt": (c_int,[_P, _P, _P, c_int, c_int, c_int, c_int, _P]),
    "frcnn_winograd_filter_transform": (c_int, [_P, c_int, c_int, _P, c_int, _P]),
    "frcnn_winograd_filter_transform_device": (c_int, [_P, c_int, c_int, c_int, c_int, _P, _P]),
    "frcnn_winograd_input_transform": (c_int, [_P, c_int, c_int, c_int, c_int, c_int, _P, _P]),
    "frcnn_winograd_output_transform": (c_int, [_P, c_int, c_int, c_int, c_int, c_int, _P, c_int, _P, _P]),
    "frcnn_winograd2_conv_x3": (c_int, [_P, c_int, c_int, c_int, _P, _P, c_int, _P, _P]),
    "frcnn_winograd7_filter_transform": (c_int, [_P, c_int, c_int, _P, _P]),
    "frcnn_winograd7_filter_transform_device": (c_int, [_P, c_int, c_int, c_int, _P, _P]),
    "frcnn_winograd7_input_transform": (c_int, [_P, c_int, c_int, _P, _P]),
    "frcnn_winograd7_output_transform": (c_int, [_P, c_int, c_int, _P, c_int, _P, _P]),
    "frcnn_winograd_input_transform_h2": (c_int, [_P, c_int, c_int, c_int, c_int, c_int, _P, _P, _P]),
    "frcnn_winograd_output_transform_h2": (c_int, [_P, c_int, c_int, c_int, c_int, c_int, _P, c_int, _P, _P, _P, _P]),
    "frcnn_winograd7_input_transform_h2": (c_int, [_P, c_int, c_int, _P, _P, _P]),
    "frcnn_winograd7_output_transform_h2": (c_int, [_P, c_int, c_int, _P, c_int, _P, _P, _P, _P]),
    "frcnn_set_tuning": (c_int, [c_int, c_int]),
    "frcnn_pack_filter_hwio": (c_int, [_P, c_int, c_int, c_int, c_int, _P, _P]),
    "frcnn_maxpool_nhwc": (c_int, [_P, c_int, c_int, c_int, c_int, c_int, c_int, c_int, c_int, _P, c_int, c_int, _P]),
    "frcnn_dwconv3x3_nhwc": (c_int, [_P, c_int, c_int, c_int, c_int, _P, _P, _P, c_int, c_int, c_int, c_int, c_int, c_int, _P]),
    "frcnn_dwconv3x3_nhwc_h2": (c_int, [_P, c_int, c_int, c_int, c_int, _P, _P, _P, _P, _P, c_int, c_int, c_int, c_int, c_int, c_int, _P]),
    "frcnn_spatial_mean": (c_int, [_P, c_int, c_int, c_int, _P, _P]),
    "frcnn_softmax_rows": (c_int, [_P, c_int, c_int, c_int, _P, _P]),
    "frcnn_rpn_softmax": (c_int, [_P, c_int, c_int, c_int, _P, _P]),
    "frcnn_copy_cols": (c_int, [_P, c_int, c_int, c_int, c_int, _P, c_int, _P]),
    "frcnn_anchor_target_workspace_bytes": (c_size_t, [c_int, c_int, c_int, c_int]),
    "frcnn_anchor_target_layer": (c_int, [_P, c_int, c_float, c_float, c_int, c_int, c_int, c_int, _P, c_int, c_double, c_double,
                                          c_double, c_longlong, _P, _P, _P, _P, _P, _P, c_size_t, _P]),
    "frcnn_anchor_target_layer_inject": (c_int, [_P, c_int, c_float, c_float, c_int, c_int, c_int, c_int, _P, c_int, c_double, c_double,
                                                 c_double, _P, c_int, _P, _P, _P, _P, _P, _P, c_size_t, _P]),
    "frcnn_proposal_target_layer_inject": (c_int, [_P, _P, c_int, _P, c_int, c_int, c_int, _P, c_int, _P, _P, _P, _P, _P, _P, _P, _P, _P, _P]),
    "frcnn_proposal_target_layer": (c_int, [_P, _P, c_int, _P, c_int, c_int, c_int, c_double, c_double, c_double, c_double, _P, _P,
                                            c_longlong, _P, _P, _P, _P, _P, _P, _P, _P, _P]),
    "frcnn_proposal_target_layer_dn": (c_int, [_P, _P, c_int, _P, _P, c_int, c_int, c_int, c_double, c_double, c_double, c_double, _P, _P,
                                               c_longlong, _P, _P, _P, _P, _P, _P, _P, _P, _P]),
    "frcnn_loss_workspace_bytes": (c_size_t, [c_longlong]),
    "frcnn_softmax_ce_loss": (c_int, [_P, _P, c_int, c_int, c_int, c_int, c_int, _P, _P, _P, c_size_t, _P]),
    "frcnn_smooth_l1_loss": (c_int, [_P, _P, _P, _P, c_longlong, c_float, c_float, _P, _P, _P, c_size_t, _P]),
    "frcnn_transpose_pad": (c_int, [_P, c_int, c_int, _P, c_int, _P]),
    "frcnn_im2col_t": (c_int, [_P, c_int, c_int, c_int, c_int, c_int, c_int, c_int, c_int, c_int, c_int, c_int, _P, c_int, _P]),
    "frcnn_flip_transpose_filter": (c_int, [_P, c_int, c_int, c_int, c_int, _P, _P]),
    "frcnn_conv2d_dgrad_strided": (c_int, [_P, c_int, c_int, c_int, c_int, _P, c_int, c_int, c_int, c_int, c_int, c_int, _P, c_int,
                                           c_int, c_int, _P]),
    "frcnn_conv2d_wgrad_supported": (c_int, [c_int, c_int]),
    "frcnn_conv2d_wgrad_workspace_bytes": (c_size_t, [c_int, c_int, c_int, c_int, c_int, c_int, c_int]),
    "frcnn_conv2d_wgrad": (c_int, [_P, _P, c_int, c_int, c_int, c_int, c_int, c_int, c_int, c_int, c_int, c_int, c_int, c_int, _P, _P,
                                   c_size_t, _P]),
    "frcnn_conv2d_wgrad_set_plan": (None, [c_int, c_int]),
    "frcnn_conv2d_wgrad_h2_workspace_bytes": (c_size_t, [c_int, c_int, c_int, c_int, c_int, c_int, c_int]),
    "frcnn_conv2d_wgrad_h2": (c_int, [_P, _P, c_int, c_int, c_int, c_int, c_int, c_int, c_int, c_int, c_int, c_int, c_int, c_int, _P, _P,
                                      c_size_t, _P]),
    "frcnn_conv2d_wgrad_h2_set_plan": (None, [c_int, c_int]),
    "frcnn_relu_bwd": (c_int, [_P, _P, c_longlong, _P]),
    "frcnn_gemm_x3_pack_bytes": (c_size_t, [c_int, c_int, c_int]),
    "frcnn_gemm_x3_pack": (c_int, [_P, c_int, c_int, c_int, _P, _P]),
    "frcnn_gemm_x3": (c_int, [_P, _P, _P, _P, _P, c_int, c_int, c_int, c_int, c_int, c_int, c_int, _P]),
    "frcnn_h2_planes_bytes": (c_size_t, [c_longlong, c_int]),
    "frcnn_h2_pack_w": (c_int, [_P, c_int, c_int, c_int, _P, _P, _P]),
    "frcnn_h2_split": (c_int, [_P, c_longlong, c_int, _P, _P, _P]),
    "frcnn_gemm_h2": (c_int, [_P, _P, _P, _P, _P, _P, _P, _P, _P, _P, _P, c_int, c_int, c_int, c_int, c_int, c_int, _P]),
    "frcnn_gemm_h2_mean_workspace_bytes": (c_size_t, [c_int, c_int, c_int]),
    "frcnn_gemm_h2_mean": (c_int, [_P, _P, _P, _P, _P, _P, _P, _P, c_int, c_int, c_int, c_int, c_int, c_int, _P, _P, c_size_t, c_int, _P]),
    "frcnn_relu6_bwd": (c_int, [_P, _P, c_longlong, _P]),
    "frcnn_maxpool_bwd": (c_int, [_P, c_int, c_int, c_int, c_int, c_int, c_int, _P, _P, c_int, c_int, _P, _P]),
    "frcnn_dropout": (c_int, [_P, c_longlong, c_ulonglong, c_float, _P, _P]),
    "frcnn_dwconv3x3_dgrad": (c_int, [_P, c_int, c_int, c_int, c_int, _P, _P, c_int, c_int, c_int, c_int, c_int, c_int, _P]),
    "frcnn_dwconv3x3_wgrad_workspace_bytes": (c_size_t, [c_int, c_int, c_int, c_int]),
    "frcnn_dwconv3x3_wgrad": (c_int, [_P, _P, c_int, c_int, c_int, c_int, c_int, c_int, c_int, c_int, c_int, _P, _P, _P, c_size_t, _P]),
    "frcnn_dwconv3x3_refold": (c_int, [_P, _P, c_int, _P, _P]),
    "frcnn_add_strided": (c_int, [_P, c_int, c_int, c_int, c_int, _P, c_int, c_int, c_int, c_int, _P]),
    "frcnn_spatial_mean_bwd": (c_int, [_P, c_int, c_int, c_int, _P, _P]),
    "frcnn_colsum": (c_int, [_P, c_int, c_int, _P, _P]),
    "frcnn_crop_and_resize_bwd": (c_int, [_P, c_int, c_int, c_int, _P, c_int, c_float, c_int, _P, _P]),
    "frcnn_crop_and_resize_bwd_plan": (c_int, [_P, c_int, c_int, c_int, _P, c_int, c_float, c_int, _P, c_size_t, _P]),
    "frcnn_sgd_momentum": (c_int, [_P, _P, _P, _P, _P, c_longlong, c_int, c_float, c_float, c_float, c_float, _P]),
    "frcnn_sgd_desc_bytes": (c_size_t, []),
    "frcnn_sgd_momentum_multi": (c_int, [_P, c_int, c_float, c_float, c_float, _P]),
    "frcnn_sgd_momentum_range": (c_int, [_P, c_int, c_int, c_float, c_float, c_float, _P]),
    "frcnn_sumsq": (c_int, [_P, c_longlong, c_double, _P, c_int, _P, c_size_t, _P]),
    "frcnn_sumsq_multi": (c_int, [_P, _P, c_int, c_double, _P, c_int, _P, c_size_t, _P]),
    "frcnn_summary_limits": (c_int, [_P]),
    "frcnn_summary_stats_workspace_bytes": (c_size_t, [c_int]),
    "frcnn_summary_stats": (c_int, [_P, c_int, _P, _P, c_size_t, _P]),
    "frcnn_graph_begin": (c_int, [_P]),
    "frcnn_graph_end": (c_int, [_P, ctypes.POINTER(c_void_p)]),
    "frcnn_graph_launch": (c_int, [_P, _P]),
    "frcnn_graph_destroy": (c_int, [_P]),
}


class FrcnnHipError(RuntimeError):
    pass


def lib():
    global _lib
    if _lib is None:
        if not os.path.exists(LIB_PATH):
# ... 31 lines not shown
```

### tf-faster-rcnn_amd/frcnn_hip/ops.py

```python
import ctypes

import numpy as np
import torch

import frcnn_hip as _binding
from . import ACT_NONE, NMS_RULE_CPU, call, check, lib

_ws_cache = {}
ws_scope = "default"

_scope_stack = [(None, None, None)]


def active_store(owner, default=None):
    o, _, store = _scope_stack[-1]
    return store if store is not None and (owner is None or o is owner) else default


def scope_depth():
    return len(_scope_stack) - 1


class unscoped(object):

# ... 1141 lines not shown
    __slots__ = ("planes", "inv", "rows", "K")

    def __init__(self, planes, inv, rows, K):
        self.planes, self.inv, self.rows, self.K = planes, inv, int(rows), int(K)

    @staticmethod
    def empty(rows, K, device):
        assert K % 128 == 0
        return H2(torch.empty(lib().frcnn_h2_planes_bytes(int(rows), int(K)), dtype=torch.uint8, device=device),
                  torch.empty((K // 128, rows), dtype=torch.float32, device=device), rows, K)

    def to_float(self):
        hl = self.planes.view(torch.float16).view(2, self.rows, self.K).float()
        inv = self.inv.t().repeat_interleave(128, dim=1)
        return (hl[0] + hl[1]) * inv


def h2_split(x, out=None):
    _chk(x)
    K = x.shape[-1]
    rows = x.numel() // K
    out = H2.empty(rows, K, x.device) if out is None else out
    assert out.rows == rows and out.K == K
    call("frcnn_h2_split", _ptr(x), rows, K, _ptr(out.planes), _ptr(out.inv), _stream())
    return out


def h2_pack_w(w, out=None):
    _chk(w)
    G, N, K = (w.shape[0], w.shape[1], w.shape[2]) if w.dim() == 3 else (1, w.shape[0], w[0].numel())
    if out is None:
        out = (torch.empty(lib().frcnn_h2_planes_bytes(G * N, K), dtype=torch.uint8, device=w.device),
               torch.empty((G, N), dtype=torch.float32, device=w.device))
    call("frcnn_h2_pack_w", _ptr(w), G, N, K, _ptr(out[0]), _ptr(out[1]), _stream())
    return out


def gemm_h2(x, wp, G, M, N, K, bias=None, residual=None, act=ACT_NONE, out=None, out_planes=None, want_f32=True, cfg=-1, mask=None):
    assert isinstance(x, H2) and x.rows == G * M and x.K == K
    if out is None and want_f32:
        out = _empty((G * M, N), dtype=torch.float32, device=x.planes.device)
    if out_planes is not None:
        assert out_planes.rows == G * M and out_planes.K == N
    rp = residual if isinstance(residual, H2) else None
    if rp is not None:
        assert rp.rows == G * M and rp.K == N
    if mask is not None:
        _chk(mask)
        assert rp is None and mask.numel() == G * M * N
        call("frcnn_gemm_h2_masked", _ptr(x.planes), _ptr(x.inv), _ptr(wp[0]), _ptr(wp[1]), _ptr(bias), _ptr(residual), _ptr(mask), _ptr(out),
             _ptr(None if out_planes is None else out_planes.planes), _ptr(None if out_planes is None else out_planes.inv),
             int(G), int(M), int(N), int(K), int(act), int(cfg), _stream())
        return out, out_planes
    call("frcnn_gemm_h2", _ptr(x.planes), _ptr(x.inv), _ptr(wp[0]), _ptr(wp[1]), _ptr(bias), _ptr(None if rp is not None else residual),
         _ptr(None if rp is None else rp.planes), _ptr(None if rp is None else rp.inv), _ptr(out),
         _ptr(None if out_planes is None else out_planes.planes), _ptr(None if out_planes is None else out_planes.inv),
         int(G), int(M), int(N), int(K), int(act), int(cfg), _stream())
    return out, out_planes


def gemm_h2_mean(x, wp, G, M, N, K, bias, residual, act, rows, out=None, cfg=-1):
    assert isinstance(x, H2) and x.rows == G * M and x.K == K and M % rows == 0
    if out is None:
        out = _empty((G * (M // rows), N), dtype=torch.float32, device=x.planes.device)
    rp = residual if isinstance(residual, H2) else None
    ws = workspace(lib().frcnn_gemm_h2_mean_workspace_bytes(int(G), int(M), int(N)), x.planes.device, "h2_mean")
    call("frcnn_gemm_h2_mean", _ptr(x.planes), _ptr(x.inv), _ptr(wp[0]), _ptr(wp[1]), _ptr(bias), _ptr(None if rp is not None else residual),
         _ptr(None if rp is None else rp.planes), _ptr(None if rp is None else rp.inv), int(G), int(M), int(N), int(K), int(act), int(rows),
         _ptr(out), _ptr(ws), ws.numel() * ws.element_size(), int(cfg), _stream())
    return out


def winograd_input_transform_h2(x, v, m):
    _chk(x)
    N, H, W, C = x.shape
    assert isinstance(v, H2) and v.K == C and v.rows == winograd_points(m) * winograd_tiles(N, H, W, m)
    if m == 7:
        call("frcnn_winograd7_input_transform_h2", _ptr(x), N, C, _ptr(v.planes), _ptr(v.inv), _stream())
    else:
        call("frcnn_winograd_input_transform_h2", _ptr(x), N, H, W, C, int(m), _ptr(v.planes), _ptr(v.inv), _stream())
    return v


def winograd_output_transform_h2(mm, bias, act, shape, m, out_planes, out=None):
    _chk(mm)
    N, H, W, C = shape
    assert isinstance(out_planes, H2) and out_planes.rows == N * H * W and out_planes.K == C
    assert mm.numel() == winograd_points(m) * winograd_tiles(N, H, W, m) * C
    if out is not None:
        _chk(out)
        assert tuple(out.shape) == tuple(shape)
    if m == 7:
        call("frcnn_winograd7_output_transform_h2", _ptr(mm), N, C, _ptr(bias), int(act), _ptr(out), _ptr(out_planes.planes),
             _ptr(out_planes.inv), _stream())
    else:
        call("frcnn_winograd_output_transform_h2", _ptr(mm), N, H, W, C, int(m), _ptr(bias), int(act), _ptr(out), _ptr(out_planes.planes),
             _ptr(out_planes.inv), _stream())
    return out_planes


def relu6_bwd(grad, y):
    _chk(grad), _chk(y)
    call("frcnn_relu6_bwd", _ptr(grad), _ptr(y), grad.numel(), _stream())
    return grad


def maxpool_bwd(x, y, dy, k, stride, dx):
    _chk(x), _chk(y), _chk(dy), _chk(dx)
    N, H, W, C = x.shape
    call("frcnn_maxpool_bwd", _ptr(x), N, H, W, C, int(k), int(stride), _ptr(y), _ptr(dy), y.shape[1], y.shape[2], _ptr(dx), _stream())
    return dx


def dropout(x, seed, keep_prob, out=None, step_mult=0):
    _chk(x)
    out = _empty(tuple(x.shape), dtype=x.dtype, device=x.device) if out is None else out
    call("frcnn_dropout", _ptr(x), x.numel(), int(seed) & 0xFFFFFFFFFFFFFFFF, float(keep_prob), _ptr(out), _stream())
    if _binding.recorder is not None and step_mult:
        _binding.recorder.patch_last(2, step_mult)
    return out


def dwconv3x3_dgrad(g, w, stride, pad, dx, accumulate=False):
    _chk(g), _chk(w), _chk(dx)
    N, OH, OW, C = g.shape
    call("frcnn_dwconv3x3_dgrad", _ptr(g), N, OH, OW, C, _ptr(w), _ptr(dx), dx.shape[1], dx.shape[2], int(stride), int(pad[0]), int(pad[2]),
         1 if accumulate else 0, _stream())
    return dx


def dwconv3x3_wgrad(g, x, stride, pad, scale, dw):
    _chk(g), _chk(x), _chk(dw)
    N, OH, OW, C = g.shape
    ws = workspace(lib().frcnn_dwconv3x3_wgrad_workspace_bytes(N, OH, OW, C), g.device, "dw_wgrad")
    call("frcnn_dwconv3x3_wgrad", _ptr(g), _ptr(x), N, x.shape[1], x.shape[2], C, OH, OW, int(stride), int(pad[0]), int(pad[2]), _ptr(scale),
         _ptr(dw), _ptr(ws), ws.numel(), _stream())
    return dw


def dwconv3x3_refold(w, scale, wf):
    _chk(w), _chk(scale), _chk(wf)
    call("frcnn_dwconv3x3_refold", _ptr(w), _ptr(scale), w.shape[-1], _ptr(wf), _stream())
    return wf


def add_strided(src, dst, stride, accumulate):
    _chk(src), _chk(dst)
    N, OH, OW, C = src.shape
    call("frcnn_add_strided", _ptr(src), N, OH, OW, C, _ptr(dst), dst.shape[1], dst.shape[2], int(stride), 1 if accumulate else 0, _stream())
    return dst


def spatial_mean_bwd(dy, HW, out):
    _chk(dy), _chk(out)
    call("frcnn_spatial_mean_bwd", _ptr(dy), dy.shape[0], int(HW), dy.shape[1], _ptr(out), _stream())
    return out


def colsum(dy2d, out):
    _chk(dy2d), _chk(out)
    call("frcnn_colsum", _ptr(dy2d), dy2d.shape[0], dy2d.shape[1], _ptr(out), _stream())
    return out


def crop_and_resize_bwd(dout, rois, feat_stride, dfeat, max_lds=0):
    _chk(dout), _chk(rois), _chk(dfeat)
# ... 119 lines not shown
```

### tf-faster-rcnn_amd/lib/model/config.py

```python
import ast
import os
import os.path as osp

import numpy as np


class AttrDict(dict):

    def __init__(self, d=None, **kw):
        super().__init__()
        for k, v in dict(d or {}, **kw).items():
            self[k] = v

    def __setitem__(self, k, v):
        if isinstance(v, dict) and not isinstance(v, AttrDict):
            v = AttrDict(v)
        super().__setitem__(k, v)

    def __getattr__(self, k):
        try:
            return self[k]
        except KeyError:
            raise AttributeError(k)

    __setattr__ = __setitem__


_TRAIN = dict(
    LEARNING_RATE=0.001, MOMENTUM=0.9, WEIGHT_DECAY=0.0001, GAMMA=0.1, STEPSIZE=[30000], DISPLAY=10,
    DOUBLE_BIAS=True, TRUNCATED=False, BIAS_DECAY=False, USE_GT=False, ASPECT_GROUPING=False,
    SNAPSHOT_KEPT=3, SUMMARY_INTERVAL=180, SCALES=(600,), MAX_SIZE=1000, IMS_PER_BATCH=1, BATCH_SIZE=128,
    FG_FRACTION=0.25, FG_THRESH=0.5, BG_THRESH_HI=0.5, BG_THRESH_LO=0.1, USE_FLIPPED=True, BBOX_REG=True,
    BBOX_THRESH=0.5, SNAPSHOT_ITERS=5000, SNAPSHOT_PREFIX='res101_faster_rcnn', BBOX_NORMALIZE_TARGETS=True,
    BBOX_INSIDE_WEIGHTS=(1.0, 1.0, 1.0, 1.0), BBOX_NORMALIZE_TARGETS_PRECOMPUTED=True,
    BBOX_NORMALIZE_MEANS=(0.0, 0.0, 0.0, 0.0), BBOX_NORMALIZE_STDS=(0.1, 0.1, 0.2, 0.2), PROPOSAL_METHOD='gt',
    HAS_RPN=True, RPN_POSITIVE_OVERLAP=0.7, RPN_NEGATIVE_OVERLAP=0.3, RPN_CLOBBER_POSITIVES=False,
    RPN_FG_FRACTION=0.5, RPN_BATCHSIZE=256, RPN_NMS_THRESH=0.7, RPN_PRE_NMS_TOP_N=12000,
    RPN_POST_NMS_TOP_N=2000, RPN_BBOX_INSIDE_WEIGHTS=(1.0, 1.0, 1.0, 1.0), RPN_POSITIVE_WEIGHT=-1.0,
    USE_ALL_GT=True)

_TEST = dict(
    SCALES=(600,), MAX_SIZE=1000, NMS=0.3, SVM=False, BBOX_REG=True, HAS_RPN=False, PROPOSAL_METHOD='gt',
    RPN_NMS_THRESH=0.7, RPN_PRE_NMS_TOP_N=6000, RPN_POST_NMS_TOP_N=300, MODE='nms', RPN_TOP_N=5000)

__C = AttrDict(
    TRAIN=_TRAIN, TEST=_TEST,
    RESNET=dict(MAX_POOL=False, FIXED_BLOCKS=1),
    MOBILENET=dict(REGU_DEPTH=False, FIXED_LAYERS=5, WEIGHT_DECAY=0.00004, DEPTH_MULTIPLIER=1.),
    PIXEL_MEANS=np.array([[[102.9801, 115.9465, 122.7717]]]), RNG_SEED=3,
    ROOT_DIR=osp.abspath(osp.join(osp.dirname(__file__), '..', '..')),
    MATLAB='matlab', EXP_DIR='default', USE_GPU_NMS=True, USE_E2E_TF=False, POOLING_MODE='crop', POOLING_SIZE=7,
    ANCHOR_SCALES=[8, 16, 32], ANCHOR_RATIOS=[0.5, 1, 2], RPN_CHANNELS=512,
    HIP=dict(WINOGRAD=True, WINOGRAD_MIN_CIN=64, WINOGRAD_M=4, WINOGRAD_F2_SCOPES=("block1", "block2"), WINOGRAD_DIRECT_SCOPES=(),
             WINOGRAD_TRAIN=True, WINOGRAD_DGRAD=True,
             WINOGRAD_7X7=True, WINOGRAD_FUSED_F2=True, FUSE_TAIL_MEAN=True, MFMA_X3=True,
             MFMA_H2=True, H2_LAZY_SPLIT=True, H2_MIN_TILES=150, H2_TRAIN_MIN_TILES=320, H2_TRUNK_PLANES=True, H2_TILE_CFG=-1,
             X3_TILE_CFG=-1, H2_TRAIN=True, WGRAD_STREAM=2, WGRAD_TN=True, WGRAD_H2=True, PREP_STREAM=True, TRAIN_REPLAY=True, TRAIN_PICK_STREAMS=6,
             GRAPH_CACHE_SHAPES=4, TRAIN_CACHE_SHAPES=16, JPEG_DEVICE=False, TEST_BATCH_IMAGES=1,
             SOFT_NMS=0, SOFT_NMS_SIGMA=0.5, SOFT_NMS_MIN_SCORE=0.001, TEST_FLIP=False, BBOX_VOTE=False, BBOX_VOTE_THRESH=0.8))
__C.DATA_DIR = osp.abspath(osp.join(__C.ROOT_DIR, 'data'))
cfg = __C


def get_output_dir(imdb, weights_filename):
    outdir = osp.abspath(osp.join(__C.ROOT_DIR, 'output', __C.EXP_DIR, imdb.name))
    outdir = osp.join(outdir, 'default' if weights_filename is None else weights_filename)
    os.makedirs(outdir, exist_ok=True)
    return outdir


def get_output_tb_dir(imdb, weights_filename):
    outdir = osp.abspath(osp.join(__C.ROOT_DIR, 'tensorboard', __C.EXP_DIR, imdb.name))
    outdir = osp.join(outdir, 'default' if weights_filename is None else weights_filename)
    os.makedirs(outdir, exist_ok=True)
    return outdir


_NULLABLE_KEYS = ("H2_TRAIN_MIN_TILES",)


def _merge_a_into_b(a, b):
    if not isinstance(a, dict):
        return
    for k, v in a.items():
        if k not in b:
            raise KeyError('{} is not a valid config key'.format(k))
        old = b[k]
        if type(old) is not type(v) and not (isinstance(old, dict) and isinstance(v, dict)):
            if isinstance(old, np.ndarray):
                v = np.array(v, dtype=old.dtype)
            elif isinstance(old, tuple) and isinstance(v, list):
                v = tuple(v)
            elif isinstance(old, list) and isinstance(v, tuple):
                v = list(v)
            elif k in _NULLABLE_KEYS and (v is None or old is None) and isinstance(old if v is None else v, int):
                pass
            else:
                raise ValueError('Type mismatch ({} vs. {}) for config key: {}'.format(type(old), type(v), k))
        if isinstance(v, dict):
            try:
                _merge_a_into_b(v, b[k])
            except Exception:
                print('Error under config key: {}'.format(k))
                raise
        else:
            b[k] = v


def cfg_from_file(filename):
    import yaml
    with open(filename, 'r') as f:
        _merge_a_into_b(AttrDict(yaml.safe_load(f) or {}), __C)


def cfg_from_list(cfg_list):
    assert len(cfg_list) % 2 == 0
    for k, v in zip(cfg_list[0::2], cfg_list[1::2]):
        path = k.split('.')
        d = __C
        for sub in path[:-1]:
            assert sub in d
            d = d[sub]
        leaf = path[-1]
        assert leaf in d
        try:
            value = ast.literal_eval(v)
        except Exception:
            value = v
        old = d[leaf]
        if isinstance(old, tuple) and isinstance(value, list):
            value = tuple(value)
        if isinstance(old, list) and isinstance(value, tuple):
            value = list(value)
        nullable = leaf in _NULLABLE_KEYS and (value is None or old is None) and isinstance(old if value is None else value, int)
        assert nullable or type(value) == type(old), 'type {} does not match original type {}'.format(type(value), type(old))
        d[leaf] = value
```

### tf-faster-rcnn_amd/lib/nets/network.py

```python
import collections

import numpy as np
import torch

from frcnn_hip import ACT_NONE, ACT_RELU, NMS_RULE_CPU, NMS_RULE_GPU, ops
from frcnn_hip.runtime import VarSpec
from model.config import cfg


class Network(object):
    def __init__(self):
        self._predictions = {}
        self._losses = {}
        self._anchor_targets = {}
        self._proposal_targets = {}
        self._layers = {}
        self._act_summaries = []
        self._variables_to_fix = {}
        self._feat_stride = [16, ]
        self._scope = "network"
        self._sess = None
        self._image = None
        self._im_info = None
        self._var_specs = collections.OrderedDict()
        self._tape = []
        self._requires_grad = set()
        self._gt_boxes = None
        self._sample_seed = 0
        self.replay_stats = dict(eager=0, recorded=0, replayed=0)
        self._replay_clock, self._train_arena, self._train_scope_key = 0, None, None
        self._train_state = None
        self._plan_batch = 0
        self._fuse_tail_entry = False
        self._h2_of = {}
        self._f32_missing = set()

    def _var(self, name, shape, init, arg=None):
        self._var_specs[name] = VarSpec(shape, init, arg)

    def _declare_conv_bn(self, scope, kh, kw, cin, cout, residual_branch_end=False):
        self._var(scope + "/weights", (kh, kw, cin, cout), "he")
        self._var(scope + "/BatchNorm/gamma", (cout,), "bn_gamma_res" if residual_branch_end else "bn_gamma")
        self._var(scope + "/BatchNorm/beta", (cout,), "bn_beta")
        self._var(scope + "/BatchNorm/moving_mean", (cout,), "bn_mean")
        self._var(scope + "/BatchNorm/moving_variance", (cout,), "bn_var")

    def _declare_conv_bias(self, scope, kh, kw, cin, cout, std):
        self._var(scope + "/weights", (kh, kw, cin, cout), "normal", std)
        self._var(scope + "/biases", (cout,), "zeros")

    def _declare_backbone(self):
        raise NotImplementedError

    def _head_channels(self):
        raise NotImplementedError

    def _tail_channels(self):
        raise NotImplementedError

    def variable_specs(self):
        return self._var_specs

    def _conv(self, x, scope, k, stride=1, pad=(0, 0, 0, 0), act=ACT_RELU, bn_eps=None, residual=None,
              res_stride=1, fold_w=False, out_affine=None, real_cin=None, no_bias=False, emit_h2=False, want_f32=True):
        sess = self._sess
        N, H, W, Cin = x.shape
        wino = (cfg.HIP.WINOGRAD and k == 3 and stride == 1 and tuple(pad) == (1, 1, 1, 1)
                and residual is None and not fold_w and out_affine is None and not no_bias
                and Cin % 32 == 0 and Cin >= cfg.HIP.WINOGRAD_MIN_CIN and act in (ACT_NONE, ACT_RELU)
                and not any(tok in scope for tok in cfg.HIP.WINOGRAD_DIRECT_SCOPES))
        if wino and self._mode == "TEST":
            return self._conv_winograd(x, scope, act, bn_eps, emit_h2, want_f32)
        wino = wino and cfg.HIP.WINOGRAD_TRAIN
        w, b = sess.conv_params(scope, bn_eps=bn_eps, fold_w=fold_w,
                                out_scale=None if out_affine is None else out_affine[0],
                                out_shift=None if out_affine is None else out_affine[1])
        if no_bias:
            b = None
        N, H, W, Cin = x.shape
        OH = ops.conv_out_size(H, k, stride, pad[0], pad[1])
        OW = ops.conv_out_size(W, k, stride, pad[2], pad[3])
        Cout = w.shape[0]
        out = sess.buf(self._tag + "/" + scope, (N, OH, OW, Cout))
        flops = 2 * N * OH * OW * Cout * k * k * (Cin if real_cin is None else real_cin)
        plain = k == 1 and stride == 1 and tuple(pad) == (0, 0, 0, 0) and not fold_w and (residual is None or res_stride == 1)
        M = N * OH * OW
        if wino:
            m = self._winograd_scheme(scope, H, W)
            G, T = ops.winograd_points(m), ops.winograd_tiles(N, H, W, m)
            u = sess.prepared.get(("fwd", "wino_u", self._tag, scope, m), lambda: ops.winograd_filter_transform_device(
                w, m, False, out=sess.buf(self._tag + "/wino_u/" + scope, (G, Cout, Cin))))
            mm = sess.buf(self._tag + "/wino_m", (G, T, Cout))
            v = sess.buf(self._tag + "/wino_v", (G, T, Cin))
            yp = sess.h2_buf(self._tag + "/" + scope, M, Cout) if (emit_h2 and cfg.HIP.MFMA_H2 and Cout % 128 == 0) else None
            sess.mark("conv:" + scope, 2 * G * T * Cout * Cin,
                      lambda: ops.conv3x3_winograd(x, u, b, act, out=out, v_buf=v, m_buf=mm, out_planes=yp),
                      nbytes=4 * (v.numel() + u.numel() + mm.numel()))
            self._wrote(out, yp, True) if yp is not None else self._wrote(out)
        elif plain and self._h2_eligible(M, Cout, Cin, 1, scope) and self._h2_input(x) is not None:
            xp, wp = self._h2_input(x), sess.h2_planes(w)
            yp = sess.h2_buf(self._tag + "/" + scope, M, Cout) if emit_h2 else None
            y = out if (want_f32 or yp is None or self._mode == "TRAIN") else None
            res = residual
            if residual is not None and residual.data_ptr() in self._f32_missing:
                res = self._h2_of[residual.data_ptr()]
            tcfg = int(cfg.HIP.H2_TILE_CFG)
            sess.mark("conv:h2:" + scope, flops, lambda: ops.gemm_h2(xp, wp, 1, M, Cout, Cin, b, res, act, out=y, out_planes=yp,
                                                                      want_f32=False, cfg=tcfg),
                      nbytes=4 * M * Cin + 4 * w.numel() + (4 * out.numel() if y is not None else 0)
                      + (4 * out.numel() if yp is not None else 0) + (4 * out.numel() if residual is not None else 0))
            self._wrote(out, yp, y is not None)
        elif plain and self._x3_eligible(M, Cout, Cin, 1):
            self._need_f32(x), self._need_f32(residual)
            planes = sess.x3_planes(w)
            xc = int(cfg.HIP.X3_TILE_CFG)
            sess.mark("conv:x3:" + scope, flops, lambda: ops.gemm_x3(x, planes, 1, M, Cout, Cin, b, residual, act, out=out, cfg=xc),
                      nbytes=4 * (x.numel() + out.numel() + (out.numel() if residual is not None else 0)) + 6 * w.numel())
            self._wrote(out)
        else:
            self._need_f32(x), self._need_f32(residual)
            sess.mark("conv:" + scope, flops,
                      lambda: ops.conv2d(x, w, b, k, k, stride, pad, act, residual, res_stride, fold_w, out=out),
                      nbytes=4 * (x.numel() + w.numel() + out.numel() + (out.numel() if residual is not None else 0)))
            self._wrote(out)
        if self._mode == "TRAIN":
            self._tape.append(dict(kind="conv", scope=scope, x=x, y=out, k=k, stride=stride, pad=tuple(pad), act=act,
                                   residual=residual, res_stride=res_stride))
            if self.trainable_scope(scope) or x.data_ptr() in self._requires_grad:
                self._requires_grad.add(out.data_ptr())
            if residual is not None and residual.data_ptr() in self._requires_grad:
                self._requires_grad.add(out.data_ptr())
        return out

    H2_MIN_CHANNEL_RATIO = 2.0 ** -18

    def _h2_eligible(self, M, N, K, G, scope=None):
        rows = G * M
        if scope is not None and self._mode == "TEST" and self._sess.h2_channel_spread(scope) < self.H2_MIN_CHANNEL_RATIO:
            return False
        return (bool(cfg.HIP.MFMA_H2) and (self._mode == "TEST" or bool(cfg.HIP.H2_TRAIN)) and K % 128 == 0 and N % 128 == 0
                and ((self._plan_rows(M) + 127) // 128) * (N // 128) * G >= self._h2_min_tiles()
                and 4 * rows * K < (1 << 32) and 4 * N * K < (1 << 32) and M * N < (1 << 29))

    @staticmethod
    def h2_min_tiles(mode):
        if mode == "TRAIN" and cfg.HIP.H2_TRAIN_MIN_TILES is not None:
            return int(cfg.HIP.H2_TRAIN_MIN_TILES)
        return int(cfg.HIP.H2_MIN_TILES)

    def _h2_min_tiles(self):
        return self.h2_min_tiles(self._mode)

    def _h2_input(self, x):
        xp = self._h2_of.get(x.data_ptr())
        if xp is None and cfg.HIP.H2_LAZY_SPLIT:
            self._need_f32(x)
            K = x.shape[-1]
            xp = self._sess.h2_buf(self._tag + "/split@%x" % x.data_ptr(), x.numel() // K, K)
            self._sess.mark("op:h2_split", 0, lambda: ops.h2_split(x, out=xp), nbytes=8 * x.numel())
            self._h2_of[x.data_ptr()] = xp
        return xp

    def _wrote(self, t, planes=None, f32=True):
        k = t.data_ptr()
        if planes is None:
            self._h2_of.pop(k, None)
        else:
            self._h2_of[k] = planes
        (self._f32_missing.discard if f32 else self._f32_missing.add)(k)
        return t

    def _need_f32(self, x):
        if x is not None and x.data_ptr() in self._f32_missing:
            raise RuntimeError("graph construction error: a float32 consumer reads a tensor that was emitted as operand planes only")

    def _x3_eligible(self, M, N, K, G):
        return (bool(cfg.HIP.MFMA_X3) and self._mode == "TEST" and N % 64 == 0 and K % 32 == 0
                and ((self._plan_rows(M) + 127) // 128) * ((N + 127) // 128) * G >= 150 and M * N < (1 << 31) and N * K < (1 << 28))

    @staticmethod
    def _winograd_scheme(scope, H, W):
        if any(tok in scope for tok in cfg.HIP.WINOGRAD_F2_SCOPES):
            return 2
        m = int(cfg.HIP.WINOGRAD_M)
        return 7 if (m == 4 and H == 7 and W == 7 and cfg.HIP.WINOGRAD_7X7) else m

    def _conv_winograd(self, x, scope, act, bn_eps, emit_h2=False, want_f32=True):
        sess = self._sess
        self._need_f32(x)
        N, H, W, Cin = x.shape
        m = self._winograd_scheme(scope, H, W)
        u, b = sess.winograd_params(scope, bn_eps=bn_eps, m=m)
        G, Cout = u.shape[0], u.shape[1]
        T = ops.winograd_tiles(N, H, W, m)
        out = sess.buf(self._tag + "/" + scope, (N, H, W, Cout))
        flops = 2 * G * T * Cout * Cin
        if (cfg.HIP.WINOGRAD_FUSED_F2 and m == 2 and Cin == 64 and Cout == 64 and self._mode == "TEST" and self._x3_eligible(T, Cout, Cin, G)
                and N * H * W < (1 << 23)):
            planes = sess.x3_planes(u)
            sess.mark("conv:x3:" + scope, flops, lambda: ops.winograd2_conv_x3(x, planes, b, act, out),
                      nbytes=4 * (x.numel() + out.numel()) + 6 * u.numel())
            return self._wrote(out)
        mm = sess.buf(self._tag + "/wino_m", (G, T, Cout))
        if self._h2_eligible(T, Cout, Cin, G, scope):
            vp, wp = sess.h2_buf(self._tag + "/wino_v", G * T, Cin), sess.h2_planes(u)
            sess.mark("op:wino_in", 0, lambda: ops.winograd_input_transform_h2(x, vp, m), nbytes=4 * (x.numel() + G * T * Cin))
            tcfg = int(cfg.HIP.H2_TILE_CFG)
            sess.mark("conv:h2:" + scope, flops, lambda: ops.gemm_h2(vp, wp, G, T, Cout, Cin, out=mm, cfg=tcfg),
                      nbytes=4 * (G * T * Cin + mm.numel()) + 4 * u.numel())
        else:
            v = sess.buf(self._tag + "/wino_v", (G, T, Cin))
            sess.mark("op:wino_in", 0, lambda: ops.winograd_input_transform(x, v, m), nbytes=4 * (x.numel() + v.numel()))
            if self._x3_eligible(T, Cout, Cin, G):
                planes = sess.x3_planes(u)
                xc = int(cfg.HIP.X3_TILE_CFG)
                sess.mark("conv:x3:" + scope, flops, lambda: ops.gemm_x3(v, planes, G, T, Cout, Cin, out=mm, cfg=xc),
                          nbytes=4 * (v.numel() + mm.numel()) + 6 * u.numel())
            else:
                sess.mark("conv:" + scope, flops, lambda: ops.gemm_batched_nt(v, u, mm), nbytes=4 * (v.numel() + u.numel() + mm.numel()))
        if emit_h2 and cfg.HIP.MFMA_H2 and Cout % 128 == 0:
            yp = sess.h2_buf(self._tag + "/" + scope, N * H * W, Cout)
            y = out if want_f32 else None
            sess.mark("op:wino_out", 0, lambda: ops.winograd_output_transform_h2(mm, b, act, (N, H, W, Cout), m, yp, y),
                      nbytes=4 * (mm.numel() + out.numel() * (2 if want_f32 else 1)))
            self._wrote(out, yp, y is not None)
        else:
            sess.mark("op:wino_out", 0, lambda: ops.winograd_output_transform(mm, b, act, out, m), nbytes=4 * (mm.numel() + out.numel()))
            self._wrote(out)
        return out

    def _conv1x1_mean(self, x, scope, group_rows, act=ACT_RELU, bn_eps=None, residual=None, name="fc7"):
        sess = self._sess
        w, b = sess.conv_params(scope, bn_eps=bn_eps)
        Cin, Cout = x.shape[-1], w.shape[0]
        rows = x.numel() // Cin
        G = max(1, self._plan_batch)
        assert rows % G == 0 and (rows // G) % group_rows == 0
        M = rows // G
        out = sess.buf(self._tag + "/" + name, (rows // group_rows, Cout))
        xp, wp = self._h2_of[x.data_ptr()], sess.h2_planes(w)
        res = residual
        if residual is not None and residual.data_ptr() in self._f32_missing:
            res = self._h2_of[residual.data_ptr()]
        tcfg = int(cfg.HIP.H2_TILE_CFG)
        sess.mark("conv:h2:" + scope, 2 * rows * Cout * Cin, lambda: ops.gemm_h2_mean(xp, wp, G, M, Cout, Cin, b, res, act, group_rows, out=out, cfg=tcfg),
                  nbytes=4 * (rows * Cin + w.numel() + out.numel() + (rows * Cout if residual is not None else 0)))
        return self._wrote(out)

    def _mean_fusable(self, rows, cout, cin, scope, group_rows=1):
        G = max(1, self._plan_batch)
        return (bool(cfg.HIP.FUSE_TAIL_MEAN) and self._mode == "TEST" and rows % G == 0 and (rows // G) % max(1, int(group_rows)) == 0
                and self._h2_eligible(rows, cout, cin, 1, scope)
                and bool(cfg.HIP.H2_LAZY_SPLIT or cfg.HIP.WINOGRAD))

    _rgb_first_conv = None

    def get_variables_to_restore(self, variables, var_keep_dic):
        skip = set(self._variables_to_fix_names())
        self._variables_to_fix = {}
        keep = []
        for name in variables:
            if name in skip:
                self._variables_to_fix[name] = True
                continue
            if name in var_keep_dic:
                keep.append(name)
        return keep

    def _variables_to_fix_names(self):
        return [] if self._rgb_first_conv is None else [self._scope + self._rgb_first_conv + "/weights"]

    def fix_variables(self, sess, pretrained_model):
        from frcnn_hip.tensor_bundle import open_checkpoint
        reader = open_checkpoint(pretrained_model)
        fixed = {}
        for name in self._variables_to_fix_names():
            fixed[name] = self._fix_one(name, reader.get_tensor(name))
        sess.load_variables(fixed)
        sess.conv_info.clear()
        return sorted(fixed)

    def _fix_one(self, name, value):
        return np.ascontiguousarray(value[:, :, ::-1, :])

    def trainable_scope(self, scope):
        return True

    def _reshape_layer(self, bottom, num_dim, name):
        raise NotImplementedError("folded into frcnn_rpn_softmax (network.py:68-78 only served the pair softmax)")

    def _softmax_layer(self, bottom, name):
        if name.startswith("rpn_cls_prob"):
            A = self._num_anchors
# ... 231 lines not shown

    _trainable_on_device = False

    @staticmethod
    def _check_supported_cfg(mode):
        t = cfg.TRAIN
        fixed = [("POOLING_MODE", cfg.POOLING_MODE, "crop")]
        bad = ["%s = %r (only %r is implemented)" % (k, v, want) for k, v, want in fixed if v != want]
        if float(t.RPN_POSITIVE_WEIGHT) >= 0 and not (0.0 < float(t.RPN_POSITIVE_WEIGHT) < 1.0):
            bad.append("TRAIN.RPN_POSITIVE_WEIGHT = %r (the reference asserts 0 < p < 1, anchor_target_layer.py:103-104)" % (t.RPN_POSITIVE_WEIGHT,))
        h = cfg.HIP
        if h.SOFT_NMS not in (0, 1, 2):
            bad.append("HIP.SOFT_NMS = %r (0 = hard NMS, 1 = linear, 2 = Gaussian)" % (h.SOFT_NMS,))
        if not float(h.SOFT_NMS_SIGMA) > 0:
            bad.append("HIP.SOFT_NMS_SIGMA = %r (must be > 0)" % (h.SOFT_NMS_SIGMA,))
        if not float(h.SOFT_NMS_MIN_SCORE) >= 0:
            bad.append("HIP.SOFT_NMS_MIN_SCORE = %r (must be >= 0)" % (h.SOFT_NMS_MIN_SCORE,))
        if not 0.0 < float(h.BBOX_VOTE_THRESH) <= 1.0:
            bad.append("HIP.BBOX_VOTE_THRESH = %r (must be in (0, 1])" % (h.BBOX_VOTE_THRESH,))
        if h.TEST_FLIP and mode == "TEST":
            bad += Network._flip_refusals()
        if bad:
            raise NotImplementedError("unsupported configuration for the HIP path: " + "; ".join(bad))

    FLIP_MAX_ROWS = 1024

    @staticmethod
    def _flip_refusals():
        bad = []
        if cfg.TEST.MODE != "nms":
            bad.append("HIP.TEST_FLIP with TEST.MODE = %r (the flip ensemble merges the 'nms' proposals of two views)" % (cfg.TEST.MODE,))
        elif 2 * int(cfg.TEST.RPN_POST_NMS_TOP_N) > Network.FLIP_MAX_ROWS:
            bad.append("HIP.TEST_FLIP with TEST.RPN_POST_NMS_TOP_N = %d (two views give %d rows per image, the post-processing holds at most %d)"
                       % (int(cfg.TEST.RPN_POST_NMS_TOP_N), 2 * int(cfg.TEST.RPN_POST_NMS_TOP_N), Network.FLIP_MAX_ROWS))
        return bad

    def create_architecture(self, mode, num_classes, tag=None, anchor_scales=(8, 16, 32), anchor_ratios=(0.5, 1, 2)):
        assert tag is not None
        self._check_supported_cfg(mode)
        if mode == "TRAIN" and not self._trainable_on_device:
            raise NotImplementedError("%s: no reverse sweep for this network's TRAIN graph; TEST mode works" % type(self).__name__)
        self._tag = tag
        self._num_classes = num_classes
        self._mode = mode
        self._anchor_scales = tuple(anchor_scales)
        self._num_scales = len(anchor_scales)
        self._anchor_ratios = tuple(anchor_ratios)
        self._num_ratios = len(anchor_ratios)
        self._num_anchors = self._num_scales * self._num_ratios
        A = self._num_anchors
        self._var_specs.clear()
        self._declare_backbone()
        hc = self._head_channels()
        self._declare_conv_bias(self._scope + "/rpn_conv/3x3", 3, 3, hc, cfg.RPN_CHANNELS, 0.01)
        self._declare_conv_bias(self._scope + "/rpn_cls_score", 1, 1, cfg.RPN_CHANNELS, 2 * A, 0.01)
        self._declare_conv_bias(self._scope + "/rpn_bbox_pred", 1, 1, cfg.RPN_CHANNELS, 4 * A, 0.01)
        tc = self._tail_channels()
        self._var(self._scope + "/cls_score/weights", (tc, num_classes), "normal", 0.01)
        self._var(self._scope + "/cls_score/biases", (num_classes,), "zeros")
        self._var(self._scope + "/bbox_pred/weights", (tc, 4 * num_classes), "normal", 0.001)
        self._var(self._scope + "/bbox_pred/biases", (4 * num_classes,), "zeros")
        names = ["rois", "rpn_cls_score", "rpn_cls_prob", "rpn_bbox_pred", "cls_score", "cls_prob", "bbox_pred"]
        return {k: k for k in names}

    def _stage_image(self, sess, image, im_info=None):
        if isinstance(image, np.ndarray):
            image = torch.from_numpy(np.ascontiguousarray(image, dtype=np.float32))
        B, H, W, C = image.shape
        if im_info is None:
            buf = sess.buf(self._tag + "/image", (B, H, W, 4), zero=True)
        else:
            with self.shape_scope(sess, (B, H, W, 4), im_info):
                buf = sess.buf(self._tag + "/image", (B, H, W, 4), zero=True)
        buf[..., :C].copy_(image, non_blocking=True)
        return buf

    def graph_key(self, image_shape, im_info):
        c = cfg[self._mode]
        return (self._tag, self._scope, self._num_classes, self._anchor_scales, self._anchor_ratios, bool(cfg.RESNET.MAX_POOL),
                bool(cfg.USE_GPU_NMS), tuple(int(v) for v in image_shape), (float(im_info[0]), float(im_info[1])), self._mode, cfg.TEST.MODE, self._fuse_tail_entry,
                c.RPN_PRE_NMS_TOP_N, c.RPN_POST_NMS_TOP_N, c.RPN_NMS_THRESH, cfg.TEST.RPN_TOP_N, cfg.POOLING_SIZE,
                bool(cfg.HIP.WINOGRAD), int(cfg.HIP.WINOGRAD_MIN_CIN), int(cfg.HIP.WINOGRAD_M), tuple(cfg.HIP.WINOGRAD_F2_SCOPES),
                tuple(cfg.HIP.WINOGRAD_DIRECT_SCOPES), bool(cfg.HIP.WINOGRAD_7X7), bool(cfg.HIP.FUSE_TAIL_MEAN), bool(cfg.HIP.MFMA_X3), bool(cfg.USE_E2E_TF),
                bool(cfg.HIP.MFMA_H2), bool(cfg.HIP.H2_LAZY_SPLIT), int(cfg.HIP.H2_MIN_TILES), bool(cfg.HIP.H2_TRUNK_PLANES), int(cfg.HIP.H2_TILE_CFG), int(cfg.HIP.X3_TILE_CFG), bool(cfg.HIP.H2_TRAIN))

    def shape_scope(self, sess, image_shape, im_info):
        return sess.shape_scope(self.graph_key(image_shape, im_info), group=("graphs", self._tag), cap=int(cfg.HIP.GRAPH_CACHE_SHAPES))

    def forward_device(self, sess, image_d, im_info, use_graph=True):
        self._sess = sess
        self._image = image_d
        self._im_info = (float(im_info[0]), float(im_info[1]), float(im_info[2]))
        sess.prepared.wait_planes()
        ops.ws_scope = self._tag
        key = self.graph_key(image_d.shape, self._im_info)
        cur = torch.cuda.current_stream(sess.device)
        with self.shape_scope(sess, image_d.shape, self._im_info):
            if not use_graph or sess.profile is not None:
                sess.flops_last_forward = 0
                self._build_network(self._mode == "TRAIN")
                return self._predictions
            if key not in sess.graphs:
                with torch.cuda.stream(sess.stream):
                    sess.stream.wait_stream(cur)
                    sess.flops_last_forward = 0
                    self._build_network(False)
                    sess.stream.synchronize()
                    flops = sess.flops_last_forward
                    g = ops.Graph().capture(lambda: self._build_network(False))
                    sess.stream.synchronize()
                sess.graphs[key] = (g, dict(self._predictions), self._num_rois, flops, self._rois_per_image, image_d)
            g, preds, num, flops, per, captured = sess.graphs[key]
            self._predictions, self._num_rois, sess.flops_last_forward, self._rois_per_image = dict(preds), num, flops, per
            if captured.data_ptr() != image_d.data_ptr():
                captured.copy_(image_d, non_blocking=True)
            g.launch()
        return self._predictions

    def _build_proposals(self):
        with self._plan_context(self, False):
            self._tape = []
            self._requires_grad = set()
            self._act_summaries = []
            self._h2_of, self._f32_missing = {}, set()
            net_conv = self._image_to_head(False)
            self._anchor_component()
            rois = self._region_proposal(net_conv, False)
        B, per, s = int(self._image.shape[0]), self._rois_per_image, self._sess
        if self._num_rois is None:
            return rois, s.buf(self._tag + "/top_scores", (per, 1)), torch.full((B,), per, dtype=torch.int32, device=rois.device)
        return rois, s.buf(self._tag + "/roi_scores", (B * per, 1)), self._num_rois

    def propose_device(self, sess, image_d, im_info, use_graph=True):
        assert self._mode == "TEST", "propose_device is a test-time path"
        self._sess = sess
        self._image = image_d
        self._im_info = (float(im_info[0]), float(im_info[1]), float(im_info[2]))
        sess.prepared.wait_planes()
        ops.ws_scope = self._tag
        scope_key = self.graph_key(image_d.shape, self._im_info)
        key = ("propose",) + scope_key
        cur = torch.cuda.current_stream(sess.device)
        with self.shape_scope(sess, image_d.shape, self._im_info):
            if not use_graph or sess.profile is not None or cfg.TEST.MODE != "nms":
                sess.flops_last_forward = 0
                return self._build_proposals()
            ent = sess.graphs.get(key)
            if ent is None:
                with torch.cuda.stream(sess.stream):
                    sess.stream.wait_stream(cur)
                    sess.flops_last_forward = 0
                    out = self._build_proposals()
                    sess.stream.synchronize()
                    flops = sess.flops_last_forward
                    g = ops.Graph().capture(self._build_proposals)
                    sess.stream.synchronize()
                ent = sess.graphs[key] = dict(scope=scope_key, graph=g, out=out, flops=flops, per=self._rois_per_image, image=image_d)
            self._num_rois, sess.flops_last_forward, self._rois_per_image = ent["out"][2], ent["flops"], ent["per"]
            if ent["image"].data_ptr() != image_d.data_ptr():
                ent["image"].copy_(image_d, non_blocking=True)
            ent["graph"].launch()
        return ent["out"]

    def extract_head(self, sess, image):
        self._sess = sess
        sess.prepared.wait_planes()
        shape = (int(image.shape[0]), int(image.shape[1]), int(image.shape[2]), 4)
# ... 346 lines not shown
```

### tf-faster-rcnn_amd/lib/nets/resnet_v1.py

```python
from frcnn_hip import ACT_NONE, ACT_RELU, ops
from model.config import cfg
from nets.network import Network

BN_EPS = 1e-5


def _same_pad(k, stride):
    total = k - 1
    beg = total // 2
    return (beg, total - beg, beg, total - beg)


class resnetv1(Network):
    _rgb_first_conv = "/conv1"
    _trainable_on_device = True
    def __init__(self, num_layers=50):
        Network.__init__(self)
        self._feat_stride = [16, ]
        self._feat_compress = [1. / float(self._feat_stride[0]), ]
        self._num_layers = num_layers
        self._scope = 'resnet_v1_%d' % num_layers
        self._decide_blocks()

    def _decide_blocks(self):
# ... 22 lines not shown
    def _head_channels(self):
        return self._blocks[2][1] * 4

    def _tail_channels(self):
        return self._blocks[3][1] * 4

    def _bottleneck(self, x, prefix, base, stride, mean_rows=0, emit_out=True, f32_out=True):
        depth = base * 4
        cin = x.shape[-1]
        if cin != depth:
            shortcut = self._conv(x, prefix + "/shortcut", 1, stride, act=ACT_NONE, bn_eps=BN_EPS)
            res_stride = 1
        else:
            shortcut, res_stride = x, stride
        r = self._conv(x, prefix + "/conv1", 1, 1, act=ACT_RELU, bn_eps=BN_EPS)
        pad = (1, 1, 1, 1) if stride == 1 else _same_pad(3, stride)
        N, H, W, _ = r.shape
        M3 = N * ops.conv_out_size(H, 3, stride, pad[0], pad[1]) * ops.conv_out_size(W, 3, stride, pad[2], pad[3])
        if mean_rows and res_stride == 1 and stride == 1 and self._mean_fusable(M3, depth, base, prefix + "/conv3", mean_rows):
            r = self._conv(r, prefix + "/conv2", 3, stride, pad, act=ACT_RELU, bn_eps=BN_EPS, emit_h2=True, want_f32=False)
            if self._h2_input(r) is not None:
                return self._conv1x1_mean(r, prefix + "/conv3", mean_rows, act=ACT_RELU, bn_eps=BN_EPS, residual=shortcut)
            x = self._conv(r, prefix + "/conv3", 1, 1, act=ACT_RELU, bn_eps=BN_EPS, residual=shortcut, res_stride=1)
            out = self._sess.buf(self._tag + "/fc7", (x.shape[0], x.shape[-1]))
            return self._sess.mark("op:spatial_mean", 0, lambda: ops.spatial_mean(x, out=out), nbytes=4 * (x.numel() + out.numel()))
        c3_h2 = res_stride == 1 and self._h2_eligible(M3, depth, base, 1, prefix + "/conv3")
        r = self._conv(r, prefix + "/conv2", 3, stride, pad, act=ACT_RELU, bn_eps=BN_EPS, emit_h2=c3_h2, want_f32=not c3_h2)
        return self._conv(r, prefix + "/conv3", 1, 1, act=ACT_RELU, bn_eps=BN_EPS, residual=shortcut, res_stride=res_stride,
                          emit_h2=emit_out, want_f32=f32_out)

    def _trunk_planes_only(self, rows, base, next_stride, next_prefix=None):
        depth = 4 * base
        return (bool(cfg.HIP.H2_TRUNK_PLANES) and next_stride == 1
                and self._h2_eligible(rows, base, depth, 1, None if next_prefix is None else next_prefix + "/conv1")
                and self._h2_eligible(rows, depth, base, 1, None if next_prefix is None else next_prefix + "/conv3"))

    def _run_blocks(self, x, blocks, emit_last=True):
        for bi, (name, base, n_units, stride) in enumerate(blocks):
            for u in range(1, n_units + 1):
                s_u = stride if u == n_units else 1
                N, H, W, _ = x.shape
                rows = N * ops.conv_out_size(H, 3, s_u, 1, 1) * ops.conv_out_size(W, 3, s_u, 1, 1) if s_u > 1 else N * H * W
                planes_only = u < n_units and self._trunk_planes_only(rows, base, stride if u + 1 == n_units else 1,
                                                                       "%s/%s/unit_%d/bottleneck_v1" % (self._scope, name, u + 1))
                x = self._bottleneck(x, "%s/%s/unit_%d/bottleneck_v1" % (self._scope, name, u), base, s_u,
                                     emit_out=emit_last or u < n_units or bi + 1 < len(blocks), f32_out=not planes_only)
        return x

    def _crop_pool_layer(self, bottom, rois, name):
        return self._crop_pool(bottom, rois, name, max_pool=bool(cfg.RESNET.MAX_POOL))

    def _build_base(self):
        net = self._conv(self._image, self._scope + "/conv1", 7, 2, _same_pad(7, 2), act=ACT_RELU, bn_eps=BN_EPS,
                         fold_w=True, real_cin=3)
        N, H, W, C = net.shape
        out = self._sess.buf(self._tag + "/pool1", (N, ops.conv_out_size(H, 3, 2, 1, 1), ops.conv_out_size(W, 3, 2, 1, 1), C))
        self._sess.mark("op:maxpool", 0, lambda: ops.maxpool(net, 3, 2, (1, 1, 1, 1), out=out), nbytes=4 * (net.numel() + out.numel()))
        return self._wrote(out)

    def _image_to_head(self, is_training, reuse=None):
        assert (0 <= cfg.RESNET.FIXED_BLOCKS <= 3)
        net_conv = self._run_blocks(self._build_base(), self._blocks[0:3])
        self._act_summaries.append(net_conv)
        self._layers['head'] = net_conv
        return net_conv

    def _fused_tail_maps(self, net_conv):
        name = self._blocks[-1][0]
        prefix = "%s/%s/unit_1/bottleneck_v1" % (self._scope, name)
        sc_map = self._conv(net_conv, prefix + "/shortcut", 1, 1, act=ACT_NONE, bn_eps=BN_EPS, no_bias=True)
        c1_map = self._conv(net_conv, prefix + "/conv1", 1, 1, act=ACT_NONE, bn_eps=BN_EPS, no_bias=True)
        return sc_map, c1_map

    def _fused_tail_entry(self, net_conv, rois):
        sess, P = self._sess, cfg.POOLING_SIZE
        name, base, n_units, stride = self._blocks[-1]
        prefix = "%s/%s/unit_1/bottleneck_v1" % (self._scope, name)
        R = rois.shape[0]
        sc_map, c1_map = self._fused_tail_maps(net_conv)
        b_sc = sess.conv_info[prefix + "/shortcut"]["b"]
        b_c1 = sess.conv_info[prefix + "/conv1"]["b"]
        fs = float(self._feat_stride[0])
        sc_out = sess.buf(self._tag + "/" + prefix + "/shortcut_crop", (R, P, P, sc_map.shape[-1]))
        c1_out = sess.buf(self._tag + "/" + prefix + "/conv1_crop", (R, P, P, c1_map.shape[-1]))
        shortcut = self._crop_images(sc_map, rois, sc_out, bias=b_sc, act=ACT_NONE)
        r = self._crop_images(c1_map, rois, c1_out, bias=b_c1, act=ACT_RELU)
        c3_h2 = self._h2_eligible(R * P * P, 4 * base, base, 1, prefix + "/conv3")
        r = self._conv(r, prefix + "/conv2", 3, 1, (1, 1, 1, 1), act=ACT_RELU, bn_eps=BN_EPS, emit_h2=c3_h2, want_f32=not c3_h2)
        x = self._conv(r, prefix + "/conv3", 1, 1, act=ACT_RELU, bn_eps=BN_EPS, residual=shortcut, res_stride=1, emit_h2=n_units >= 2,
                       want_f32=not (n_units >= 2 and self._trunk_planes_only(R * P * P, base, stride if n_units == 2 else 1,
                                                                              "%s/%s/unit_2/bottleneck_v1" % (self._scope, name))))
        fused = stride == 1 and n_units >= 2 and self._mean_fusable(R * P * P, 4 * base, base, "%s/%s/unit_%d/bottleneck_v1/conv3" % (self._scope, name, n_units), P * P)
        for u in range(2, n_units + 1):
            x = self._bottleneck(x, "%s/%s/unit_%d/bottleneck_v1" % (self._scope, name, u), base, stride if u == n_units else 1,
                                 mean_rows=P * P if (fused and u == n_units) else 0, emit_out=u < n_units,
                                 f32_out=not (u < n_units and self._trunk_planes_only(R * P * P, base, stride if u + 1 == n_units else 1,
                                                                                      "%s/%s/unit_%d/bottleneck_v1" % (self._scope, name, u + 1))))
        if fused:
            return x
        out = sess.buf(self._tag + "/fc7", (x.shape[0], x.shape[-1]))
        return sess.mark("op:spatial_mean", 0, lambda: ops.spatial_mean(x, out=out), nbytes=4 * (x.numel() + out.numel()))

    def _head_to_tail(self, pool5, is_training, reuse=None):
        name, base, n_units, stride = self._blocks[-1]
        if stride == 1 and self._mean_fusable(pool5.shape[0] * pool5.shape[1] * pool5.shape[2], 4 * base, base,
                                              "%s/%s/unit_%d/bottleneck_v1/conv3" % (self._scope, name, n_units), pool5.shape[1] * pool5.shape[2]):
            x = pool5
            hw = pool5.shape[1] * pool5.shape[2]
            for u in range(1, n_units + 1):
                x = self._bottleneck(x, "%s/%s/unit_%d/bottleneck_v1" % (self._scope, name, u), base, 1, mean_rows=hw if u == n_units else 0)
            return x
        fc7 = self._run_blocks(pool5, self._blocks[-1:], emit_last=False)
        out = self._sess.buf(self._tag + "/fc7", (fc7.shape[0], fc7.shape[-1]))
        res = self._sess.mark("op:spatial_mean", 0, lambda: ops.spatial_mean(fc7, out=out), nbytes=4 * (fc7.numel() + out.numel()))
        if self._mode == "TRAIN":
            self._tape.append(dict(kind="mean", x=fc7, y=res, name=self._scope + "/fc7_mean"))
            if fc7.data_ptr() in self._requires_grad:
                self._requires_grad.add(res.data_ptr())
        return res

    def trainable_scope(self, scope):
        fixed = ["/conv1"] + ["/block%d/" % b for b in range(1, cfg.RESNET.FIXED_BLOCKS + 1)]
        tail = scope[len(self._scope):]
        return not any(tail.startswith(f) for f in fixed)
```

Measured before the change: 555.3.

## Fuse ROI crop-and-resize into Winograd 7x7 input transform for tail conv2

Adds a kernel that samples the bilinear ROI crop of the conv1 map, applies bias and ReLU, and writes the Winograd F(7) input transform directly as fp16 planes. The tail entry uses it, so the intermediate crop tensor is never written and read back and one launch is dropped. It also adds an option to route conv3 GEMMs that take a planes residual to a different pipelined tile config, plus a scratch timing script. The risks are lower occupancy or poorer memory access in the fused kernel, and exact-equivalence of the crop arithmetic, which the script checks.

```diff
diff --git a/include/frcnn_hip.h b/include/frcnn_hip.h
--- a/include/frcnn_hip.h
+++ b/include/frcnn_hip.h
@@ -221,6 +221,9 @@
 int frcnn_winograd7_input_transform_h2(const float* x_d, int R, int C, void* v_planes_d, float* v_inv_d, void* stream);
 int frcnn_winograd7_output_transform_h2(const float* m_d, int R, int C, const float* bias_d, int act, float* y_d, void* y_planes_d,
                                         float* y_inv_d, void* stream);
+int frcnn_winograd7_input_transform_h2_crop(const float* feat_d, int N, int H, int W, int C, const float* rois_d, int R,
+                                            float feat_stride, const float* bias_d, int act, void* v_planes_d, float* v_inv_d,
+                                            void* stream);
 int frcnn_pack_filter_hwio(const float* w_hwio, int KH, int KW, int Cin, int Cout, const float* scale, float* out);
 int frcnn_maxpool_nhwc(const float* x_d, int N, int H, int W, int C, int k, int stride, int pad_top,
                        int pad_left, float* y_d, int OH, int OW, void* stream);
diff --git a/scratch/tail_entry_time.py b/scratch/tail_entry_time.py
--- /dev/null
+++ b/scratch/tail_entry_time.py
@@ -0,0 +1,121 @@
+import os
+import sys
+
+import numpy as np
+import torch
+
+ROOT = os.path.dirname(os.path.dirname(os.path.abspath(__file__)))
+PKG = os.path.join(ROOT, "tf-faster-rcnn_amd")
+for p in (ROOT, PKG, os.path.join(PKG, "lib")):
+    sys.path.insert(0, p)
+import frcnn_hip
+from frcnn_hip import ops
+
+log = open(sys.argv[1] if len(sys.argv) > 1 else os.devnull, "w")
+
+
+def say(s):
+    print(s, flush=True)
+    log.write(s + "\n")
+    log.flush()
+
+
+def time_variants(variants, rounds=50, warm=5):
+    ev = {n: [] for n in variants}
+    for r in range(warm + rounds):
+        for n, fn in variants.items():
+            a, b = torch.cuda.Event(enable_timing=True), torch.cuda.Event(enable_timing=True)
+            a.record()
+            fn()
+            b.record()
+            b.synchronize()
+            if r >= warm:
+                ev[n].append(a.elapsed_time(b) * 1000.0)
+    return {n: (float(np.median(v)), float(np.min(v))) for n, v in ev.items()}
+
+
+dev = torch.device("cuda:0")
+torch.cuda.set_device(0)
+L = frcnn_hip.lib()
+g = torch.Generator(device=dev)
+g.manual_seed(1)
+
+NIMG, H, W, C, R = 8, 38, 63, 512, 2400
+feat = torch.randn(NIMG, H, W, C, device=dev, generator=g)
+bias = torch.randn(C, device=dev, generator=g)
+rng = np.random.RandomState(2)
+rois = np.zeros((R, 5), dtype=np.float32)
+per = R // NIMG
+for i in range(R):
+    w, h = rng.uniform(30, 600), rng.uniform(30, 450)
+    x1, y1 = rng.uniform(0, 1000 - w), rng.uniform(0, 600 - h)
+    rois[i] = (i // per, x1, y1, x1 + w, y1 + h)
+rois_d = torch.from_numpy(rois).to(dev)
+crop = torch.empty(R, 7, 7, C, device=dev)
+v2 = ops.H2.empty(121 * R, C, dev)
+vf = ops.H2.empty(121 * R, C, dev)
+
+
+def two_launches():
+    ops.crop_and_resize_bias_act(feat, rois_d, 16.0, 7, bias, 1, out=crop)
+    ops.winograd_input_transform_h2(crop, v2, 7)
+
+
+def crop_only():
+    ops.crop_and_resize_bias_act(feat, rois_d, 16.0, 7, bias, 1, out=crop)
+
+
+def transform_only():
+    ops.winograd_input_transform_h2(crop, v2, 7)
+
+
+def fused(order):
+    def f():
+        L.frcnn_set_tuning(10, order)
+        ops.winograd7_input_transform_h2_crop(feat, rois_d, 16.0, bias, 1, vf)
+    return f
+
+
+two_launches()
+for order in (0, 1):
+    vf.planes.fill_(0)
+    vf.inv.fill_(0)
+    fused(order)()
+    torch.cuda.synchronize()
+    say("full size, order %d: planes equal %s, scales equal %s" % (order, torch.equal(vf.planes, v2.planes), torch.equal(vf.inv, v2.inv)))
+t = time_variants({"crop+transform": two_launches, "crop": crop_only, "transform": transform_only,
+                   "fused group-fast": fused(0), "fused roi-per-workgroup": fused(1)})
+L.frcnn_set_tuning(10, 0)
+say("Part 1 (R 2400, C 512, map 8 x 38 x 63), us median / min over 50 alternating rounds")
+for n, (med, mn) in t.items():
+    say("  %-26s %8.1f %8.1f" % (n, med, mn))
+del crop, v2, vf, feat
+torch.cuda.empty_cache()
+
+M, K, N = 117600, 512, 2048
+x = torch.randn(M, K, device=dev, generator=g).clamp_(min=0)
+wt = torch.randn(N, K, device=dev, generator=g) / K ** 0.5
+b = torch.randn(N, device=dev, generator=g)
+res = torch.randn(M, N, device=dev, generator=g).clamp_(min=0)
+xp, wp, rp = ops.h2_split(x), ops.h2_pack_w(wt), ops.h2_split(res)
+del x, res
+torch.cuda.empty_cache()
+outs = {c: ops.H2.empty(M, N, dev) for c in (31, 34, 40)}
+
+
+def conv3(c):
+    def f():
+        ops.gemm_h2(xp, wp, 1, M, N, K, b, rp, 1, out=None, out_planes=outs[c], want_f32=False, cfg=c)
+    return f
+
+
+for c in outs:
+    conv3(c)()
+torch.cuda.synchronize()
+say("conv3 planes: cfg 34 == cfg 31: %s / %s; cfg 40 == cfg 31: %s" % (torch.equal(outs[34].planes, outs[31].planes),
+                                                                   torch.equal(outs[34].inv, outs[31].inv), torch.equal(outs[40].planes, outs[31].planes)))
+t = time_variants({"cfg 31": conv3(31), "cfg 34": conv3(34), "cfg 40": conv3(40)})
+say("Part 2 (planes residual, planes out, M 117600, K 512, N 2048), us median / min over 50 alternating rounds")
+for n, (med, mn) in t.items():
+    say("  %-26s %8.1f %8.1f" % (n, med, mn))
+log.close()
diff --git a/tf-faster-rcnn_amd/csrc/conv_igemm.hip b/tf-faster-rcnn_amd/csrc/conv_igemm.hip
--- a/tf-faster-rcnn_amd/csrc/conv_igemm.hip
+++ b/tf-faster-rcnn_amd/csrc/conv_igemm.hip
@@ -555,7 +555,9 @@
 static thread_local int g_plan_images = 0;
 static constexpr int PLAN_IMAGES = 4;
 extern thread_local int g_wino_rows_below;
+extern thread_local int g_wino7_crop_order;
 extern "C" int frcnn_set_tuning(int key, int value) {
+  if (key == 10) { g_wino7_crop_order = value ? 1 : 0; return FRCNN_OK; }
   if (key == 9) { g_wino_rows_below = value > 0 ? value : 256; return FRCNN_OK; }
   if (key == 0) { g_force_cfg = value; return FRCNN_OK; }
   if (key == 5) { g_stagger = value; return FRCNN_OK; }
diff --git a/tf-faster-rcnn_amd/csrc/crop_math.h b/tf-faster-rcnn_amd/csrc/crop_math.h
--- /dev/null
+++ b/tf-faster-rcnn_amd/csrc/crop_math.h
@@ -0,0 +1,50 @@
+#pragma once
+#include "common.h"
+
+__device__ __forceinline__ float4 lerp4(const float4 a, const float4 b, float t) {
+  return make_float4(a.x + (b.x - a.x) * t, a.y + (b.y - a.y) * t, a.z + (b.z - a.z) * t, a.w + (b.w - a.w) * t);
+}
+__device__ __forceinline__ float2 lerp2(const float2 a, const float2 b, float t) {
+  return make_float2(a.x + (b.x - a.x) * t, a.y + (b.y - a.y) * t);
+}
+
+struct CropGeom { float x1, y1, hs, ws; };
+__device__ __forceinline__ CropGeom crop_geom(const float* __restrict__ roi, int H, int W, float stride, int P) {
+  const float height = ((float)H - 1.0f) * stride, width = ((float)W - 1.0f) * stride;
+  const float x1 = roi[1] / width, y1 = roi[2] / height, x2 = roi[3] / width, y2 = roi[4] / height;
+  CropGeom g;
+  g.x1 = x1; g.y1 = y1;
+  g.hs = (y2 - y1) * (float)(H - 1) / (float)(P - 1);
+  g.ws = (x2 - x1) * (float)(W - 1) / (float)(P - 1);
+  return g;
+}
+
+struct CropAxis { int lo, hi; float t; bool in; };
+__device__ __forceinline__ CropAxis crop_axis(float start, float step, int g, int n) {
+  const float p = start * (float)(n - 1) + (float)g * step;
+  CropAxis a;
+  a.in = p >= 0 && p <= (float)(n - 1);
+  a.lo = a.in ? (int)floorf(p) : 0;
+  a.hi = a.in ? (int)ceilf(p) : 0;
+  a.t = p - (float)a.lo;
+  return a;
+}
+
+__device__ __forceinline__ float4 crop_sample(const float4* __restrict__ feat, int H, int W, int C4, int c4, float y1,
+                                              float x1, float hs, float ws, int gy, int gx) {
+  const float in_y = y1 * (float)(H - 1) + (float)gy * hs;
+  const float in_x = x1 * (float)(W - 1) + (float)gx * ws;
+  if (in_y < 0 || in_y > (float)(H - 1) || in_x < 0 || in_x > (float)(W - 1)) return make_float4(0, 0, 0, 0);
+  const int top = (int)floorf(in_y), bot = (int)ceilf(in_y);
+  const int left = (int)floorf(in_x), right = (int)ceilf(in_x);
+  const float ly = in_y - (float)top, lx = in_x - (float)left;
+  const float4 tl = feat[((size_t)top * W + left) * C4 + c4], tr = feat[((size_t)top * W + right) * C4 + c4];
+  const float4 bl = feat[((size_t)bot * W + left) * C4 + c4], br = feat[((size_t)bot * W + right) * C4 + c4];
+  return lerp4(lerp4(tl, tr, lx), lerp4(bl, br, lx), ly);
+}
+
+__device__ __forceinline__ float2 crop_blend2(const float2 tl, const float2 tr, const float2 bl, const float2 br, const CropAxis& y,
+                                              const CropAxis& x) {
+  const float2 v = lerp2(lerp2(tl, tr, x.t), lerp2(bl, br, x.t), y.t);
+  return (y.in && x.in) ? v : make_float2(0.f, 0.f);
+}
diff --git a/tf-faster-rcnn_amd/csrc/detect_kernels.hip b/tf-faster-rcnn_amd/csrc/detect_kernels.hip
--- a/tf-faster-rcnn_amd/csrc/detect_kernels.hip
+++ b/tf-faster-rcnn_amd/csrc/detect_kernels.hip
@@ -1,6 +1,7 @@
 #include "common.h"
 #include "softnms_math.h"
 #include "boxvote_math.h"
+#include "crop_math.h"
 
 extern "C" int frcnn_generate_anchors(int base_size, const double* ratios, int n_ratios, const double* scales,
                                       int n_scales, double* out_base) {
@@ -819,24 +820,8 @@
                                          nms_thresh, rois_d, scores_d, num_d, ws, ws_bytes, stream);
 }
 
-__device__ __forceinline__ float4 lerp4(const float4 a, const float4 b, float t) {
-  return make_float4(a.x + (b.x - a.x) * t, a.y + (b.y - a.y) * t, a.z + (b.z - a.z) * t, a.w + (b.w - a.w) * t);
-}
 __device__ __forceinline__ float4 max4(const float4 a, const float4 b) {
   return make_float4(fmaxf(a.x, b.x), fmaxf(a.y, b.y), fmaxf(a.z, b.z), fmaxf(a.w, b.w));
-}
-
-__device__ __forceinline__ float4 crop_sample(const float4* __restrict__ feat, int H, int W, int C4, int c4, float y1,
-                                              float x1, float hs, float ws, int gy, int gx) {
-  const float in_y = y1 * (float)(H - 1) + (float)gy * hs;
-  const float in_x = x1 * (float)(W - 1) + (float)gx * ws;
-  if (in_y < 0 || in_y > (float)(H - 1) || in_x < 0 || in_x > (float)(W - 1)) return make_float4(0, 0, 0, 0);
-  const int top = (int)floorf(in_y), bot = (int)ceilf(in_y);
-  const int left = (int)floorf(in_x), right = (int)ceilf(in_x);
-  const float ly = in_y - (float)top, lx = in_x - (float)left;
-  const float4 tl = feat[((size_t)top * W + left) * C4 + c4], tr = feat[((size_t)top * W + right) * C4 + c4];
-  const float4 bl = feat[((size_t)bot * W + left) * C4 + c4], br = feat[((size_t)bot * W + right) * C4 + c4];
-  return lerp4(lerp4(tl, tr, lx), lerp4(bl, br, lx), ly);
 }
 
 template <bool MAX2>
@@ -846,7 +831,6 @@
   const int slab = blockIdx.x % nslab, rp = blockIdx.x / nslab;
   const int r = rp / pool, py = rp % pool;
   const int SC4 = C4 / nslab, c40 = slab * SC4;
-  const float height = ((float)H - 1.0f) * stride, width = ((float)W - 1.0f) * stride;
   const float* roi = rois + 5 * (size_t)r;
   const int img = (int)roi[0];
   float4* orow = out + ((size_t)r * pool + py) * pool * C4;
@@ -855,10 +839,8 @@
     return;
   }
   const float4* feat = feat_all + (size_t)img * H * W * C4;
-  const float x1 = roi[1] / width, y1 = roi[2] / height, x2 = roi[3] / width, y2 = roi[4] / height;
-  const int P = MAX2 ? 2 * pool : pool;
-  const float hs = (y2 - y1) * (float)(H - 1) / (float)(P - 1);
-  const float ws = (x2 - x1) * (float)(W - 1) / (float)(P - 1);
+  const CropGeom g = crop_geom(roi, H, W, stride, MAX2 ? 2 * pool : pool);
+  const float x1 = g.x1, y1 = g.y1, hs = g.hs, ws = g.ws;
   for (int t = threadIdx.x; t < pool * SC4; t += 256) {
     const int px = t / SC4, c4 = c40 + t % SC4;
     float4 v;
@@ -885,7 +867,6 @@
                                                              const float4* __restrict__ bias, int act, float4* __restrict__ out) {
   const int slab = blockIdx.x % nslab, r = blockIdx.x / nslab;
   const int SC4 = C4 / nslab, c40 = slab * SC4;
-  const float height = ((float)H - 1.0f) * stride, width = ((float)W - 1.0f) * stride;
   const float* roi = rois + 5 * (size_t)r;
   const int img = (int)roi[0];
   float4* obase = out + (size_t)r * pool * pool * C4;
@@ -895,10 +876,8 @@
     return;
   }
   const float4* feat = feat_all + (size_t)img * H * W * C4;
-  const float x1 = roi[1] / width, y1 = roi[2] / height, x2 = roi[3] / width, y2 = roi[4] / height;
-  const int P = MAX2 ? 2 * pool : pool;
-  const float hs = (y2 - y1) * (float)(H - 1) / (float)(P - 1);
-  const float ws = (x2 - x1) * (float)(W - 1) / (float)(P - 1);
+  const CropGeom g = crop_geom(roi, H, W, stride, MAX2 ? 2 * pool : pool);
+  const float x1 = g.x1, y1 = g.y1, hs = g.hs, ws = g.ws;
   for (int t0 = threadIdx.x; t0 < total; t0 += 256 * ITEMS) {
     float4 v[ITEMS];
 #pragma unroll
diff --git a/tf-faster-rcnn_amd/csrc/gemm_h2.hip b/tf-faster-rcnn_amd/csrc/gemm_h2.hip
--- a/tf-faster-rcnn_amd/csrc/gemm_h2.hip
+++ b/tf-faster-rcnn_amd/csrc/gemm_h2.hip
@@ -1156,8 +1156,8 @@
 static int run_h2(GemmH2Params& p, int cfg, hipStream_t st) {
   const int G = p.batch, M = p.M, N = p.N, K = p.K;
   if (cfg < 0) {
-    const bool classes = cfg == -1;
-    if (cfg == -9) cfg = -1;
+    const bool classes = cfg == -1 || cfg == -10, planesres_pp = (FRCNN_H2_PP_CLASSES & 8) || cfg == -10;
+    if (cfg == -9 || cfg == -10) cfg = -1;
     const long long mt256 = (M + 255) / 256, t256 = mt256 * (N / 128) * G;
 #ifndef FRCNN_H2_PP_MIN_K
 #define FRCNN_H2_PP_MIN_K 1024
@@ -1175,6 +1175,8 @@
       if (conv3_f32res && !pp) pp_cfg = 34;
       pp = pp || products || conv3_f32res;
       to31 = (FRCNN_H2_PP_CLASSES & 4) && p.resp && p.yp && !p.y && K == 512;
+      const bool conv3_planesres = planesres_pp && p.resp && p.yp && !p.y && K == 512 && waste64_ok && t256 >= 256;
+      if (conv3_planesres && !pp) { pp_cfg = 34; pp = true; to31 = false; }
     }
     const bool tiny = (long long)((M + 127) / 128) * (N / 128) * G < 150;
     const bool de = cfg != -2 && cfg != -7 && !p.mean_part && !p.mask && ((p.resp && p.yp && !p.y) || cfg == -8) && !to31;
diff --git a/tf-faster-rcnn_amd/csrc/winograd7.hip b/tf-faster-rcnn_amd/csrc/winograd7.hip
--- a/tf-faster-rcnn_amd/csrc/winograd7.hip
+++ b/tf-faster-rcnn_amd/csrc/winograd7.hip
@@ -1,4 +1,5 @@
 #include "h2_common.h"
+#include "crop_math.h"
 
 namespace w7 {
 constexpr float BT[11][9] = {
@@ -55,6 +56,33 @@
 };
 
 template <bool H2>
+__device__ __forceinline__ void wino7_input_points(const float2 (&d)[7][7], int r, int R, int c2, int C2, const Wino7Sink<H2>& V) {
+#pragma unroll
+  for (int xi = 0; xi < 11; ++xi) {
+    float2 t[7];
+#pragma unroll
+    for (int j = 0; j < 7; ++j) {
+      bool first = true;
+      t[j] = make_float2(0.f, 0.f);
+#pragma unroll
+      for (int i = 0; i < 7; ++i) acc_term(t[j], first, w7::BT[xi][i + 1], d[i][j]);
+    }
+    float2 o[11];
+    size_t rw[11];
+#pragma unroll
+    for (int nu = 0; nu < 11; ++nu) {
+      bool first = true;
+      float2 v = make_float2(0.f, 0.f);
+#pragma unroll
+      for (int j = 0; j < 7; ++j) acc_term(v, first, w7::BT[nu][j + 1], t[j]);
+      o[nu] = v;
+      rw[nu] = (size_t)(xi * 11 + nu) * R + r;
+    }
+    V.template putn<11>(rw, o, c2, C2);
+  }
+}
+
+template <bool H2>
 __global__ void __launch_bounds__(256) k_wino7_input(const float2* __restrict__ x, int R, int C2, const Wino7Sink<H2> V) {
   const long long id = (long long)blockIdx.x * blockDim.x + threadIdx.x;
   if (id >= (long long)R * C2) return;
@@ -66,29 +94,70 @@
   for (int i = 0; i < 7; ++i)
 #pragma unroll
     for (int j = 0; j < 7; ++j) d[i][j] = src[(size_t)(i * 7 + j) * C2];
-#pragma unroll
-  for (int xi = 0; xi < 11; ++xi) {
-    float2 t[7];
-#pragma unroll
-    for (int j = 0; j < 7; ++j) {
-      bool first = true;
-      t[j] = make_float2(0.f, 0.f);
-#pragma unroll
-      for (int i = 0; i < 7; ++i) acc_term(t[j], first, w7::BT[xi][i + 1], d[i][j]);
-    }
-    float2 o[11];
-    size_t rw[11];
-#pragma unroll
-    for (int nu = 0; nu < 11; ++nu) {
-      bool first = true;
-      float2 v = make_float2(0.f, 0.f);
-#pragma unroll
-      for (int j = 0; j < 7; ++j) acc_term(v, first, w7::BT[nu][j + 1], t[j]);
-      o[nu] = v;
-      rw[nu] = (size_t)(xi * 11 + nu) * R + r;
-    }
-    V.template putn<11>(rw, o, c2, C2);
-  }
+  wino7_input_points<H2>(d, r, R, c2, C2, V);
+}
+
+__device__ __forceinline__ int uni(int v) { return __builtin_amdgcn_readfirstlane(v); }
+__device__ __forceinline__ float uni(float v) { return __uint_as_float(__builtin_amdgcn_readfirstlane(__float_as_uint(v))); }
+__device__ __forceinline__ CropAxis uni(const CropAxis a) {
+  CropAxis u;
+  u.lo = uni(a.lo); u.hi = uni(a.hi); u.t = uni(a.t); u.in = uni((int)a.in) != 0;
+  return u;
+}
+
+template <bool GROUP_FAST>
+__global__ void __launch_bounds__(256) k_wino7_input_crop(const float2* __restrict__ feat_all, int NIMG, int H, int W, int C2,
+                                                           const float* __restrict__ rois, int R, float stride,
+                                                           const float2* __restrict__ bias, int act, const Wino7Sink<true> V) {
+  const int groups = C2 >> 6, wave = threadIdx.x >> 6, lane = threadIdx.x & 63;
+  int r, grp;
+  if (GROUP_FAST) {
+    grp = blockIdx.x % groups;
+    r = (blockIdx.x / groups) * 4 + wave;
+  } else {
+    const long long w = (long long)blockIdx.x * 4 + wave;
+    grp = (int)(w % groups);
+    r = (int)(w / groups);
+  }
+  r = uni(r);
+  if (r >= R) return;
+  const int c2 = uni(grp) * 64 + lane;
+  const float* roi = rois + 5 * (size_t)r;
+  const int img = uni((int)roi[0]);
+  float2 d[7][7];
+  if (img < 0 || img >= NIMG) {
+#pragma unroll
+    for (int i = 0; i < 7; ++i)
+#pragma unroll
+      for (int j = 0; j < 7; ++j) d[i][j] = make_float2(0.f, 0.f);
+  } else {
+    const float2* feat = feat_all + (size_t)img * H * W * C2 + c2;
+    const CropGeom g = crop_geom(roi, H, W, stride, 7);
+    const float2 bv = bias ? bias[c2] : make_float2(0.f, 0.f);
+    CropAxis ax[7];
+#pragma unroll
+    for (int j = 0; j < 7; ++j) ax[j] = uni(crop_axis(g.x1, g.ws, j, W));
+#pragma unroll
+    for (int i = 0; i < 7; ++i) {
+      const CropAxis ay = uni(crop_axis(g.y1, g.hs, i, H));
+      const float2* top = feat + (size_t)ay.lo * W * C2;
+      const float2* bot = feat + (size_t)ay.hi * W * C2;
+      float2 tl[7], tr[7], bl[7], br[7];
+#pragma unroll
+      for (int j = 0; j < 7; ++j) {
+        tl[j] = top[(size_t)ax[j].lo * C2]; tr[j] = top[(size_t)ax[j].hi * C2];
+        bl[j] = bot[(size_t)ax[j].lo * C2]; br[j] = bot[(size_t)ax[j].hi * C2];
+      }
+#pragma unroll
+      for (int j = 0; j < 7; ++j) {
+        float2 v = crop_blend2(tl[j], tr[j], bl[j], br[j], ay, ax[j]);
+        if (bias) v = make_float2(v.x + bv.x, v.y + bv.y);
+        if (act == FRCNN_ACT_RELU) v = act_relu(v);
+        d[i][j] = v;
+      }
+    }
+  }
+  wino7_input_points<true>(d, r, R, c2, C2, V);
 }
 
 template <int XI0, int NXI, int I0, int NI, bool H2, bool MASK>
@@ -219,6 +288,28 @@
   return FRCNN_OK;
 }
 
+thread_local int g_wino7_crop_order = 0;
+
+extern "C" int frcnn_winograd7_input_transform_h2_crop(const float* feat_d, int NIMG, int H, int W, int C, const float* rois_d, int R,
+                                                       float feat_stride, const float* bias_d, int act, void* v_planes_d, float* v_inv_d,
+                                                       void* stream) {
+  if (!feat_d || !rois_d || !v_planes_d || !v_inv_d || NIMG <= 0 || H < 2 || W < 2 || C <= 0 || R <= 0) return FRCNN_E_ARG;
+  if (act != FRCNN_ACT_NONE && act != FRCNN_ACT_RELU) return FRCNN_E_ARG;
+  if (C % H2_KB) return FRCNN_E_UNSUPPORTED;
+  const int C2 = C / 2, groups = C2 / 64;
+  const long long blocks = g_wino7_crop_order == 0 ? (long long)((R + 3) / 4) * groups : ((long long)R * groups + 3) / 4;
+  if (blocks >= (1ll << 31)) return FRCNN_E_UNSUPPORTED;
+  const Wino7Sink<true> sink{nullptr, (unsigned short*)v_planes_d, v_inv_d, (size_t)121 * R};
+  if (g_wino7_crop_order == 0)
+    hipLaunchKernelGGL(k_wino7_input_crop<true>, dim3((unsigned)blocks), dim3(256), 0, (hipStream_t)stream, (const float2*)feat_d, NIMG, H, W, C2,
+                       rois_d, R, feat_stride, (const float2*)bias_d, act, sink);
+  else
+    hipLaunchKernelGGL(k_wino7_input_crop<false>, dim3((unsigned)blocks), dim3(256), 0, (hipStream_t)stream, (const float2*)feat_d, NIMG, H, W, C2,
+                       rois_d, R, feat_stride, (const float2*)bias_d, act, sink);
+  LAUNCH_CHECK();
+  return FRCNN_OK;
+}
+
 extern "C" int frcnn_winograd7_output_transform(const float* m_d, int R, int C, const float* bias_d, int act, float* y_d, void* stream) {
   if (!m_d || !y_d || R <= 0 || C <= 0) return FRCNN_E_ARG;
   if (C % 2 || (act != FRCNN_ACT_NONE && act != FRCNN_ACT_RELU)) return FRCNN_E_UNSUPPORTED;
diff --git a/tf-faster-rcnn_amd/frcnn_hip/__init__.py b/tf-faster-rcnn_amd/frcnn_hip/__init__.py
--- a/tf-faster-rcnn_amd/frcnn_hip/__init__.py
+++ b/tf-faster-rcnn_amd/frcnn_hip/__init__.py
@@ -111,6 +111,7 @@
     "frcnn_winograd_input_transform_h2": (c_int, [_P, c_int, c_int, c_int, c_int, c_int, _P, _P, _P]),
     "frcnn_winograd_output_transform_h2": (c_int, [_P, c_int, c_int, c_int, c_int, c_int, _P, c_int, _P, _P, _P, _P]),
     "frcnn_winograd7_input_transform_h2": (c_int, [_P, c_int, c_int, _P, _P, _P]),
+    "frcnn_winograd7_input_transform_h2_crop": (c_int, [_P, c_int, c_int, c_int, c_int, _P, c_int, c_float, _P, c_int, _P, _P, _P]),
     "frcnn_winograd7_output_transform_h2": (c_int, [_P, c_int, c_int, _P, c_int, _P, _P, _P, _P]),
     "frcnn_set_tuning": (c_int, [c_int, c_int]),
     "frcnn_pack_filter_hwio": (c_int, [_P, c_int, c_int, c_int, c_int, _P, _P]),
diff --git a/tf-faster-rcnn_amd/frcnn_hip/ops.py b/tf-faster-rcnn_amd/frcnn_hip/ops.py
--- a/tf-faster-rcnn_amd/frcnn_hip/ops.py
+++ b/tf-faster-rcnn_amd/frcnn_hip/ops.py
@@ -1247,6 +1247,16 @@
     return v
 
 
+def winograd7_input_transform_h2_crop(feat, rois, feat_stride, bias, act, v):
+    _chk(feat), _chk(rois)
+    N, H, W, C = feat.shape
+    R = rois.shape[0]
+    assert isinstance(v, H2) and v.K == C and v.rows == winograd_points(7) * R
+    call("frcnn_winograd7_input_transform_h2_crop", _ptr(feat), N, H, W, C, _ptr(rois), R, float(feat_stride), _ptr(bias), int(act),
+         _ptr(v.planes), _ptr(v.inv), _stream())
+    return v
+
+
 def winograd_output_transform_h2(mm, bias, act, shape, m, out_planes, out=None):
     _chk(mm)
     N, H, W, C = shape
diff --git a/tf-faster-rcnn_amd/lib/model/config.py b/tf-faster-rcnn_amd/lib/model/config.py
--- a/tf-faster-rcnn_amd/lib/model/config.py
+++ b/tf-faster-rcnn_amd/lib/model/config.py
@@ -53,7 +53,7 @@
     ANCHOR_SCALES=[8, 16, 32], ANCHOR_RATIOS=[0.5, 1, 2], RPN_CHANNELS=512,
     HIP=dict(WINOGRAD=True, WINOGRAD_MIN_CIN=64, WINOGRAD_M=4, WINOGRAD_F2_SCOPES=("block1", "block2"), WINOGRAD_DIRECT_SCOPES=(),
              WINOGRAD_TRAIN=True, WINOGRAD_DGRAD=True,
-             WINOGRAD_7X7=True, WINOGRAD_FUSED_F2=True, FUSE_TAIL_MEAN=True, MFMA_X3=True,
+             WINOGRAD_7X7=True, WINOGRAD_FUSED_F2=True, WINO7_CROP_INPUT=True, FUSE_TAIL_MEAN=True, MFMA_X3=True,
              MFMA_H2=True, H2_LAZY_SPLIT=True, H2_MIN_TILES=150, H2_TRAIN_MIN_TILES=320, H2_TRUNK_PLANES=True, H2_TILE_CFG=-1,
              X3_TILE_CFG=-1, H2_TRAIN=True, WGRAD_STREAM=2, WGRAD_TN=True, WGRAD_H2=True, PREP_STREAM=True, TRAIN_REPLAY=True, TRAIN_PICK_STREAMS=6,
              GRAPH_CACHE_SHAPES=4, TRAIN_CACHE_SHAPES=16, JPEG_DEVICE=False, TEST_BATCH_IMAGES=1,
diff --git a/tf-faster-rcnn_amd/lib/nets/network.py b/tf-faster-rcnn_amd/lib/nets/network.py
--- a/tf-faster-rcnn_amd/lib/nets/network.py
+++ b/tf-faster-rcnn_amd/lib/nets/network.py
@@ -65,10 +65,8 @@
               res_stride=1, fold_w=False, out_affine=None, real_cin=None, no_bias=False, emit_h2=False, want_f32=True):
         sess = self._sess
         N, H, W, Cin = x.shape
-        wino = (cfg.HIP.WINOGRAD and k == 3 and stride == 1 and tuple(pad) == (1, 1, 1, 1)
-                and residual is None and not fold_w and out_affine is None and not no_bias
-                and Cin % 32 == 0 and Cin >= cfg.HIP.WINOGRAD_MIN_CIN and act in (ACT_NONE, ACT_RELU)
-                and not any(tok in scope for tok in cfg.HIP.WINOGRAD_DIRECT_SCOPES))
+        wino = (residual is None and not fold_w and out_affine is None and not no_bias
+                and self._winograd_route(scope, k, stride, pad, Cin, act))
         if wino and self._mode == "TEST":
             return self._conv_winograd(x, scope, act, bn_eps, emit_h2, want_f32)
         wino = wino and cfg.HIP.WINOGRAD_TRAIN
@@ -179,16 +177,30 @@
                 and ((self._plan_rows(M) + 127) // 128) * ((N + 127) // 128) * G >= 150 and M * N < (1 << 31) and N * K < (1 << 28))
 
     @staticmethod
+    def _winograd_route(scope, k, stride, pad, Cin, act):
+        return bool(cfg.HIP.WINOGRAD and k == 3 and stride == 1 and tuple(pad) == (1, 1, 1, 1)
+                    and Cin % 32 == 0 and Cin >= cfg.HIP.WINOGRAD_MIN_CIN and act in (ACT_NONE, ACT_RELU)
+                    and not any(tok in scope for tok in cfg.HIP.WINOGRAD_DIRECT_SCOPES))
+
+    def _wino7_crop_route(self, scope, R, Cin, Cout, act):
+        P = cfg.POOLING_SIZE
+        return (bool(cfg.HIP.WINO7_CROP_INPUT) and self._mode == "TEST" and P == 7
+                and self._winograd_route(scope, 3, 1, (1, 1, 1, 1), Cin, act) and self._winograd_scheme(scope, P, P) == 7
+                and self._h2_eligible(ops.winograd_tiles(R, P, P, 7), Cout, Cin, ops.winograd_points(7), scope))
+
+    @staticmethod
     def _winograd_scheme(scope, H, W):
         if any(tok in scope for tok in cfg.HIP.WINOGRAD_F2_SCOPES):
             return 2
         m = int(cfg.HIP.WINOGRAD_M)
         return 7 if (m == 4 and H == 7 and W == 7 and cfg.HIP.WINOGRAD_7X7) else m
 
-    def _conv_winograd(self, x, scope, act, bn_eps, emit_h2=False, want_f32=True):
+    def _conv_winograd(self, x, scope, act, bn_eps, emit_h2=False, want_f32=True, crop=None):
         sess = self._sess
         self._need_f32(x)
         N, H, W, Cin = x.shape
+        if crop is not None:
+            N, H, W = crop[0].shape[0], cfg.POOLING_SIZE, cfg.POOLING_SIZE
         m = self._winograd_scheme(scope, H, W)
         u, b = sess.winograd_params(scope, bn_eps=bn_eps, m=m)
         G, Cout = u.shape[0], u.shape[1]
@@ -204,11 +216,18 @@
         mm = sess.buf(self._tag + "/wino_m", (G, T, Cout))
         if self._h2_eligible(T, Cout, Cin, G, scope):
             vp, wp = sess.h2_buf(self._tag + "/wino_v", G * T, Cin), sess.h2_planes(u)
-            sess.mark("op:wino_in", 0, lambda: ops.winograd_input_transform_h2(x, vp, m), nbytes=4 * (x.numel() + G * T * Cin))
+            if crop is not None:
+                assert m == 7
+                rois, cb, cact = crop
+                fs = float(self._feat_stride[0])
+                sess.mark("op:wino_in", 0, lambda: ops.winograd7_input_transform_h2_crop(x, rois, fs, cb, cact, vp), nbytes=4 * (x.numel() + G * T * Cin))
+            else:
+                sess.mark("op:wino_in", 0, lambda: ops.winograd_input_transform_h2(x, vp, m), nbytes=4 * (x.numel() + G * T * Cin))
             tcfg = int(cfg.HIP.H2_TILE_CFG)
             sess.mark("conv:h2:" + scope, flops, lambda: ops.gemm_h2(vp, wp, G, T, Cout, Cin, out=mm, cfg=tcfg),
                       nbytes=4 * (G * T * Cin + mm.numel()) + 4 * u.numel())
         else:
+            assert crop is None
             v = sess.buf(self._tag + "/wino_v", (G, T, Cin))
             sess.mark("op:wino_in", 0, lambda: ops.winograd_input_transform(x, v, m), nbytes=4 * (x.numel() + v.numel()))
             if self._x3_eligible(T, Cout, Cin, G):
@@ -606,7 +625,7 @@
                 c.RPN_PRE_NMS_TOP_N, c.RPN_POST_NMS_TOP_N, c.RPN_NMS_THRESH, cfg.TEST.RPN_TOP_N, cfg.POOLING_SIZE,
                 bool(cfg.HIP.WINOGRAD), int(cfg.HIP.WINOGRAD_MIN_CIN), int(cfg.HIP.WINOGRAD_M), tuple(cfg.HIP.WINOGRAD_F2_SCOPES),
                 tuple(cfg.HIP.WINOGRAD_DIRECT_SCOPES), bool(cfg.HIP.WINOGRAD_7X7), bool(cfg.HIP.FUSE_TAIL_MEAN), bool(cfg.HIP.MFMA_X3), bool(cfg.USE_E2E_TF),
-                bool(cfg.HIP.MFMA_H2), bool(cfg.HIP.H2_LAZY_SPLIT), int(cfg.HIP.H2_MIN_TILES), bool(cfg.HIP.H2_TRUNK_PLANES), int(cfg.HIP.H2_TILE_CFG), int(cfg.HIP.X3_TILE_CFG), bool(cfg.HIP.H2_TRAIN))
+                bool(cfg.HIP.MFMA_H2), bool(cfg.HIP.H2_LAZY_SPLIT), int(cfg.HIP.H2_MIN_TILES), bool(cfg.HIP.H2_TRUNK_PLANES), int(cfg.HIP.H2_TILE_CFG), int(cfg.HIP.X3_TILE_CFG), bool(cfg.HIP.H2_TRAIN), bool(cfg.HIP.WINO7_CROP_INPUT))
 
     def shape_scope(self, sess, image_shape, im_info):
         return sess.shape_scope(self.graph_key(image_shape, im_info), group=("graphs", self._tag), cap=int(cfg.HIP.GRAPH_CACHE_SHAPES))
diff --git a/tf-faster-rcnn_amd/lib/nets/resnet_v1.py b/tf-faster-rcnn_amd/lib/nets/resnet_v1.py
--- a/tf-faster-rcnn_amd/lib/nets/resnet_v1.py
+++ b/tf-faster-rcnn_amd/lib/nets/resnet_v1.py
@@ -128,11 +128,14 @@
         b_c1 = sess.conv_info[prefix + "/conv1"]["b"]
         fs = float(self._feat_stride[0])
         sc_out = sess.buf(self._tag + "/" + prefix + "/shortcut_crop", (R, P, P, sc_map.shape[-1]))
-        c1_out = sess.buf(self._tag + "/" + prefix + "/conv1_crop", (R, P, P, c1_map.shape[-1]))
         shortcut = self._crop_images(sc_map, rois, sc_out, bias=b_sc, act=ACT_NONE)
-        r = self._crop_images(c1_map, rois, c1_out, bias=b_c1, act=ACT_RELU)
         c3_h2 = self._h2_eligible(R * P * P, 4 * base, base, 1, prefix + "/conv3")
-        r = self._conv(r, prefix + "/conv2", 3, 1, (1, 1, 1, 1), act=ACT_RELU, bn_eps=BN_EPS, emit_h2=c3_h2, want_f32=not c3_h2)
+        if self._wino7_crop_route(prefix + "/conv2", R, c1_map.shape[-1], base, ACT_RELU):
+            r = self._conv_winograd(c1_map, prefix + "/conv2", ACT_RELU, BN_EPS, emit_h2=c3_h2, want_f32=not c3_h2, crop=(rois, b_c1, ACT_RELU))
+        else:
+            c1_out = sess.buf(self._tag + "/" + prefix + "/conv1_crop", (R, P, P, c1_map.shape[-1]))
+            r = self._crop_images(c1_map, rois, c1_out, bias=b_c1, act=ACT_RELU)
+            r = self._conv(r, prefix + "/conv2", 3, 1, (1, 1, 1, 1), act=ACT_RELU, bn_eps=BN_EPS, emit_h2=c3_h2, want_f32=not c3_h2)
         x = self._conv(r, prefix + "/conv3", 1, 1, act=ACT_RELU, bn_eps=BN_EPS, residual=shortcut, res_stride=1, emit_h2=n_units >= 2,
                        want_f32=not (n_units >= 2 and self._trunk_planes_only(R * P * P, base, stride if n_units == 2 else 1,
                                                                               "%s/%s/unit_2/bottleneck_v1" % (self._scope, name))))
```

Result: no change. 558.2, median of 6 (+0.5%).
